# themeshpotato/rust-ray-tracing-in-a-weekend

Hardware: AMD Instinct MI355X
Metric: Msamples/s (pixels x spp) for 1200x800 random-spheres scene (higher is better)
Workload: dtype f64

## Files before the change

__graft_entry__.py:

```python
from __future__ import annotations

import concurrent.futures as cf
import importlib.util
import os
import subprocess
import sys

REPO = os.path.dirname(os.path.abspath(__file__))
PKG = os.path.join(REPO, "rust-ray-tracing-in-a-weekend_amd")
CSRC = os.path.join(PKG, "csrc")
INCLUDE = os.path.join(REPO, "include")
ORACLE = os.path.join(REPO, "oracle")

HIPCC = os.environ.get("HIPCC", "/opt/rocm/bin/hipcc")
ARCH = os.environ.get("RT_OFFLOAD_ARCH", "gfx950")
CXXFLAGS = ["-O3", "-std=c++17", "-fPIC", "-ffp-contract=off", "-fno-fast-math", f"--offload-arch={ARCH}",
            "-I" + INCLUDE, "-Wall", "-Wno-unused-function",
            "-mllvm", "-disable-machine-licm"]
F32_FLAGS = ["-ffp-contract=fast"]
F32_SPHERES_FLAGS = ["-fno-hip-fp32-correctly-rounded-divide-sqrt"]
F32_FINAL_FLAGS = ["-fno-hip-fp32-correctly-rounded-divide-sqrt"]


def tu_flags(src: str, flags=None) -> list:
    flags = list(CXXFLAGS if flags is None else flags)
    name = os.path.basename(src)
    if name.startswith("trace_f32_"):
        flags = [f for f in flags if f != "-ffp-contract=off"] + F32_FLAGS
        if name.startswith("trace_f32_spheres"):
            flags += F32_SPHERES_FLAGS
        if name.startswith("trace_f32_final"):
            flags += F32_FINAL_FLAGS
    return flags


VARIANTS = ["all", "final", "media", "rectinst", "spheres"]
SOURCES = ([f"trace_v_{v}.hip" for v in VARIANTS] + [f"trace_v_{v}_count.hip" for v in VARIANTS] +
           [f"trace_f32_{v}.hip" for v in VARIANTS] + ["trace_f32_final_count.hip", "trace_f32_spheres_count.hip"] +
           [f"features_v_{v}.hip" for v in VARIANTS] +
           ["trace_kernel.hip", "features_kernel.hip", "adaptive_kernel.hip", "adaptive_state_kernel.hip", "denoise_kernel.hip", "atrous_kernel.hip", "cross_kernel.hip", "pyramid_kernel.hip", "scene_model.cpp", "flatten.cpp", "bvh_build.cpp", "scene_lower.cpp",
            "launch_plan.cpp", "deal_cache.cpp", "denoise_host.cpp", "atrous_host.cpp", "cross_host.cpp", "pyramid_host.cpp", "abi.cpp", "abi_scene.cpp",
            "abi_passes.cpp", "abi_adaptive_state.cpp", "adaptive_frame.cpp", "adaptive_schedule.cpp", "abi_filters.cpp", "comm.cpp"])


def _run(cmd):
    r = subprocess.run(cmd, capture_output=True, text=True)
    if r.returncode != 0:
        raise RuntimeError(f"command failed ({r.returncode}): {' '.join(cmd)}\n{r.stdout}\n{r.stderr}")
    return r


def build_library(verbose: bool = False, extra_flags=(), name: str = "librtiow_amd.so", licm: bool = False,
                  csrc: str = CSRC) -> str:
    objdir = os.path.join(PKG, "build" if not (extra_flags or licm or csrc != CSRC) else "build_" + os.path.splitext(name)[0])
    flags = [f for f in CXXFLAGS if not (licm and f in ("-mllvm", "-disable-machine-licm"))]
    libdir = os.path.join(PKG, "lib")
    os.makedirs(objdir, exist_ok=True)
    os.makedirs(libdir, exist_ok=True)

    ident = [f'-DRT_SRC_HASH="{source_hash(extra_flags, licm=licm, csrc=csrc)}"']

    stamp = os.path.join(objdir, "flags.txt")
    flag_line = " ".join(flags + list(extra_flags)) + " | f32: " + " ".join(F32_FLAGS) + " | f32 spheres: " + \
        " ".join(F32_SPHERES_FLAGS) + " | f32 final: " + " ".join(F32_FINAL_FLAGS)
    same_flags = os.path.exists(stamp) and open(stamp).read() == flag_line
    headers = [os.path.join(csrc, f) for f in os.listdir(csrc) if f.endswith(".hpp")] + \
              [os.path.join(INCLUDE, "rt", f) for f in os.listdir(os.path.join(INCLUDE, "rt"))]
    newest_header = max(os.path.getmtime(h) for h in headers)

    def compile_one(src):
        obj = os.path.join(objdir, os.path.splitext(src)[0] + ".o")
        path = os.path.join(csrc, src)
        if (same_flags and src != "abi.cpp" and os.path.exists(obj) and
                os.path.getmtime(obj) > max(os.path.getmtime(path), newest_header)):
            return obj
        lang = [] if src.endswith(".hip") else ["-x", "hip"]
        _run([HIPCC, *lang, *tu_flags(src, flags), *extra_flags, *(ident if src == "abi.cpp" else []), "-c", path,
              "-o", obj])
        return obj

    with cf.ThreadPoolExecutor(max_workers=min(8, os.cpu_count() or 4)) as ex:
        objs = list(ex.map(compile_one, SOURCES))
    open(stamp, "w").write(flag_line)
    out = os.path.join(libdir, name)
    _run([HIPCC, f"--offload-arch={ARCH}", "-shared", "-o", out, *objs, "-ldl"])
    if verbose:
        print("built", out)
    return out


def source_hash(extra_flags=(), licm: bool = False, csrc: str = CSRC) -> str:
    import hashlib
    flags = [f for f in CXXFLAGS if not f.startswith("-I") and not (licm and f in ("-mllvm", "-disable-machine-licm"))]
    h = hashlib.sha256(" ".join(flags + list(extra_flags) + F32_FLAGS + F32_SPHERES_FLAGS + F32_FINAL_FLAGS).encode())
    for d in (csrc, os.path.join(INCLUDE, "rt")):
        for name in sorted(os.listdir(d)):
            if name.endswith((".hip", ".hpp", ".cpp", ".h")):
                h.update(name.encode())
                h.update(open(os.path.join(d, name), "rb").read())
    return h.hexdigest()[:16]


SAN_FLAGS = ["-Xarch_host", "-fsanitize=address", "-Xarch_host", "-fsanitize=undefined",
             "-Xarch_host", "-fno-sanitize-recover=undefined", "-Xarch_host", "-fno-omit-frame-pointer"]
HOST_SOURCES = ["scene_model.cpp", "flatten.cpp", "bvh_build.cpp", "scene_lower.cpp", "launch_plan.cpp", "deal_cache.cpp",
                "denoise_host.cpp", "atrous_host.cpp", "cross_host.cpp", "pyramid_host.cpp", "abi.cpp", "abi_scene.cpp", "abi_passes.cpp",
                "abi_adaptive_state.cpp", "adaptive_frame.cpp", "adaptive_schedule.cpp", "abi_filters.cpp",
                "comm.cpp"]


def build_sanitized() -> tuple:
    objdir = os.path.join(PKG, "build")
    kernel_objs = [os.path.join(objdir, os.path.splitext(s)[0] + ".o") for s in SOURCES if s not in HOST_SOURCES]
    if not all(os.path.exists(o) for o in kernel_objs):
        build_library()
    sandir = os.path.join(PKG, "build_asan")
    os.makedirs(sandir, exist_ok=True)

    ident = [f'-DRT_SRC_HASH="{source_hash()}"']

    def compile_one(src):
        obj = os.path.join(sandir, os.path.splitext(src)[0] + ".o")
        _run([HIPCC, "-x", "hip", *CXXFLAGS, "-O1", "-g", *SAN_FLAGS, *(ident if src == "abi.cpp" else []), "-c",
              os.path.join(CSRC, src), "-o", obj])
        return obj

    with cf.ThreadPoolExecutor(max_workers=3) as ex:
        objs = list(ex.map(compile_one, HOST_SOURCES))
    lib = os.path.join(PKG, "lib", "librtiow_amd_asan.so")
    _run([HIPCC, f"--offload-arch={ARCH}", "-shared", "-o", lib, *objs, *kernel_objs, "-ldl"])
    _run(["make", "-C", ORACLE, "-s", "asan"])
    return lib, os.path.join(ORACLE, "build", "liboracle_asan.so")


def build_oracle() -> str:
    _run(["make", "-C", ORACLE, "-s"])
    return os.path.join(ORACLE, "build", "liboracle.so")


def import_binding():
    if PKG not in sys.path:
        sys.path.insert(0, PKG)
    spec = importlib.util.spec_from_file_location("rtiow_amd", os.path.join(PKG, "rtiow_amd.py"))
    mod = importlib.util.module_from_spec(spec)
    sys.modules["rtiow_amd"] = mod
    spec.loader.exec_module(mod)
    return mod


def build_calib() -> str:
    for name in ("valu_calib", "write_calib"):
        src = os.path.join(REPO, "scripts", "calib", name + ".hip")
        out = os.path.join(REPO, "scripts", "calib", name)
        _run([HIPCC, "-O3", f"--offload-arch={ARCH}", src, "-o", out])
    return os.path.join(REPO, "scripts", "calib", "valu_calib")


def build() -> None:
    build_library()
    build_oracle()
    build_calib()
    rt = import_binding()
    lib = rt.load_library()
    missing = [s for s in rt.EXPORTED if not hasattr(lib, s)]
    if missing:
        raise RuntimeError(f"library is missing exports: {missing}")


def smoke() -> None:
    import numpy as np
    sys.path.insert(0, REPO)
    rt = import_binding()
    from tests import oracle_binding as ob

    W, H, spp = 48, 32, 4
    img, stats = rt.render_scene(0, W, H, spp, max_depth=50, out_format=rt.RT_OUT_F64)
    ref = ob.render(0, W, H, spp, max_depth=50)
    err = float(np.max(np.abs(img - ref)))
    print(f"smoke: random scene {W}x{H}x{spp}: kernel {stats.kernel_ms:.3f} ms, max |gpu - oracle| = {err:.3e}")
    if not err <= 1e-3:
        raise AssertionError(f"GPU render differs from the oracle: L_inf = {err}")


if __name__ == "__main__":
    cmd = sys.argv[1] if len(sys.argv) > 1 else "build"
    {"build": build, "smoke": smoke}[cmd]()
```

include/rt/rt_abi.h:

```cpp
#ifndef RT_ABI_H
#define RT_ABI_H

#include <stddef.h>
#include <stdint.h>

#include "rt_scene.h"

#ifdef __cplusplus
extern "C" {
#endif

#define RT_ABI_VERSION 6

enum {
    RT_OK = 0,
    RT_ERR_INVALID = -1,
    RT_ERR_HIP = -2,
    RT_ERR_UNSUPPORTED = -3,
    RT_ERR_OOM = -4,
    RT_ERR_NO_DEVICE = -5,
    RT_ERR_NO_SCENE = -6,
    RT_ERR_COMM = -7,
    RT_ERR_PEER = -8
};
// ... 53 lines not shown
typedef struct rt_scene_preset {
    double look_from[3], look_at[3], background[3];
    double vfov, aperture, focus_dist, time0, time1;
    int32_t default_width, default_spp;
    double default_aspect;
} rt_scene_preset;
int rt_scene_preset_get(int scene_id, rt_scene_preset* out);
int rt_scene_camera(int scene_id, int width, int height, rt_camera* cam_out, double background_out[3]);

enum {
    RT_BUILD_C_ISECT = 1,
    RT_BUILD_MAX_LEAF = 2,
    RT_BUILD_FORCE_LEAF = 3,
    RT_BUILD_ROOT_LEAF = 4,
    RT_BUILD_SPLIT_BOX_PAIRS = 5,
    RT_BUILD_SPLIT_BLAS_PAIRS = 6,
    RT_BUILD_TIME0 = 7,
    RT_BUILD_TIME1 = 8
};
int rt_world_set_build_option(rt_world* w, int key, double value);
int rt_world_flatten(rt_world* w, int accel, const rt_scene_soa** soa_out);
int rt_scene_validate(const rt_scene_soa* soa, int32_t* tlas_depth, int32_t* blas_depth);
int rt_ctx_upload_soa(rt_ctx* ctx, const rt_scene_soa* soa);
int rt_ctx_upload_world(rt_ctx* ctx, rt_world* w, int accel);

enum { RT_OUT_F32 = 0, RT_OUT_F64 = 1 };

typedef struct rt_render_params {
    int32_t width, height;
    int32_t spp, max_depth;
    int32_t spp_chunk;
    int32_t row_begin, row_stride;
    int32_t out_format;
    int32_t out_on_device;
    int32_t count_work;
    double background[3];
    uint64_t render_seed;
    void* stream;
    int32_t row_block;
    int32_t tile_shard;
} rt_render_params;

int rt_render(rt_ctx* ctx, const rt_camera* cam, const rt_render_params* p, void* out);

int rt_rows_in_shard(int height, int row_begin, int row_stride);
int rt_rows_in_band_shard(int height, int row_begin, int row_stride, int row_block);
int rt_tiles_in_shard(int width, int height, int tile_begin, int tile_stride);

typedef struct rt_stats {
    double kernel_ms;
    double reduce_ms;
    uint64_t samples;
    uint64_t casts;
    uint64_t node_visits;
    uint64_t prim_tests;
    uint64_t n_items;
    int32_t n_chunks, spp_chunk;
    int64_t scene_bytes;
    int32_t node_bytes, prim_bytes, material_bytes;
    int32_t variant_features;
    int32_t slab32;
    int32_t lds_stack;
    int32_t lds_nodes;
    uint64_t cycles_camera;
    uint64_t cycles_trace;
    uint64_t cycles_shade;
    uint64_t wave_steps;
    uint64_t wave_node_steps;
    uint64_t cycles_nodes;
    uint64_t cycles_leaves;
    int32_t schedule;
    int32_t n_batches;
    uint64_t wave_leaf_steps;
    uint64_t camera_lanes;
    uint64_t camera_steps;
    uint64_t shade_lanes;
    uint64_t shade_steps;
    int32_t precision;
    int32_t waves_per_simd;
    int64_t trace_buf_bytes;
    int32_t overlapped;
    int32_t reserved0;
    int64_t ring_bytes;
} rt_stats;
int rt_last_stats(rt_ctx* ctx, rt_stats* out);
int rt_last_counters(rt_ctx* ctx, uint64_t* out, int n);

int rt_last_tile_costs(rt_ctx* ctx, uint64_t* out, int64_t n);
int rt_ctx_set_tile_order(rt_ctx* ctx, const uint32_t* order, int64_t n);
int rt_last_deal_order(rt_ctx* ctx, uint32_t* out, int64_t n);

typedef struct rt_comm rt_comm;
enum { RT_COMM_ID_BYTES = 128 };
int rt_comm_unique_id(uint8_t id[RT_COMM_ID_BYTES]);
int rt_comm_init_rank(rt_ctx* ctx, int rank, int world, const uint8_t id[RT_COMM_ID_BYTES], rt_comm** out);
int rt_comm_init_all(rt_ctx* const* ctxs, int n, rt_comm** comms_out);
void rt_comm_destroy(rt_comm* comm);
int rt_comm_rank(const rt_comm* comm, int* rank, int* world);

int rt_comm_tile_order(rt_comm* comm, const rt_camera* cam, const rt_render_params* p, int cost_spp);
int rt_comm_tile_order_all(rt_comm* const* comms, int n, const rt_camera* cam, const rt_render_params* p,
                           int cost_spp);

int rt_render_gather(rt_comm* comm, const rt_camera* cam, const rt_render_params* p, void* frame);
int rt_render_gather_all(rt_comm* const* comms, int n, const rt_camera* cam, const rt_render_params* p,
                         void* frame);

typedef struct rt_comm_stats {
    double render_ms;
    double gather_ms;
    double assemble_ms;
    double kernel_ms;
    int64_t slab_bytes;
    int32_t tiles;
    int32_t tile_order;
    double cost_pass_ms;
    int32_t peer_failed;
} rt_comm_stats;
int rt_comm_last_stats(rt_comm* comm, rt_comm_stats* out);

int rt_tiles_assemble(rt_ctx* ctx, const void* slabs, int64_t slab_elems, int world, const rt_render_params* p,
                      void* frame);
int rt_tiles_assemble_host(const void* slabs, int64_t slab_elems, int world, int width, int height, int elem_bytes,
                           const uint32_t* order, void* frame);
int rt_cost_tile_order(const uint64_t* costs, int64_t n, uint32_t* order);

typedef struct rt_accum rt_accum;
int rt_accum_create(rt_ctx* ctx, const rt_render_params* p, rt_accum** out);
void rt_accum_destroy(rt_accum* acc);
int rt_accum_add(rt_ctx* ctx, rt_accum* acc, const rt_camera* cam, const rt_render_params* p, int sample_count);
int rt_accum_get(rt_accum* acc, double* sums, int64_t* samples_done);
int rt_accum_set(rt_accum* acc, const double* sums, int64_t samples_done);
int rt_accum_resolve(rt_ctx* ctx, rt_accum* acc, double divisor, int out_format, int out_on_device, void* out);

typedef int (*rt_progress_fn)(void* user, int64_t samples_done, int64_t samples_total);
int rt_render_progressive(rt_ctx* ctx, const rt_camera* cam, const rt_render_params* p, int batch_spp,
                          rt_progress_fn progress, void* user, void* out);

typedef struct rt_adaptive_params {
    int32_t min_spp;
    int32_t step_spp;
    double threshold;
} rt_adaptive_params;

typedef struct rt_adaptive_out {
    void* mean;
    uint32_t* tile_spp;
    double* tile_error;
    double* stderr_map;
} rt_adaptive_out;

int rt_render_adaptive(rt_ctx* ctx, const rt_camera* cam, const rt_render_params* p, const rt_adaptive_params* ap,
                       const rt_adaptive_out* out);

typedef struct rt_adaptive_stats {
    int32_t passes;
    int32_t min_spp, step_spp;
    int32_t spp_chunk;
    int32_t tiles;
    int32_t max_pass_batches;
    uint64_t samples_traced;
    uint64_t samples_uniform;
    double trace_ms;
    double moments_ms;
    double classify_ms;
} rt_adaptive_stats;
int rt_adaptive_last_stats(rt_ctx* ctx, rt_adaptive_stats* out);

// ... 111 lines not shown
    double sigma_albedo, sigma_normal, sigma_depth;
} rt_denoise_guides;
int rt_denoise_guided(rt_ctx* ctx, const rt_denoise_params* p, const void* mean, const double* stderr_map,
                      const rt_denoise_guides* g, void* out);
int rt_denoise_guided_host(const rt_denoise_params* p, const void* mean, const double* stderr_map,
                           const rt_denoise_guides* g, void* out);

typedef struct rt_atrous_params {
    int32_t width, height, format, on_device;
    int32_t levels, demodulate;
    double sigma_l;
    void* stream;
} rt_atrous_params;
int rt_denoise_atrous(rt_ctx* ctx, const rt_atrous_params* p, const void* mean, const double* stderr_map,
                      const rt_denoise_guides* g, void* out, double* stderr_out );
int rt_denoise_atrous_host(const rt_atrous_params* p, const void* mean, const double* stderr_map,
                           const rt_denoise_guides* g, void* out, double* stderr_out );

typedef struct rt_atrous_stats {
    double kernel_ms;
    int32_t levels;
    int64_t scratch_bytes;
} rt_atrous_stats;
int rt_atrous_last_stats(rt_ctx* ctx, rt_atrous_stats* out);

typedef struct rt_cross_params {
    int32_t width, height, format, on_device;
    int32_t radius, patch;
    double k;
    double variance_scale;
    void* stream;
} rt_cross_params;
int rt_denoise_cross(rt_ctx* ctx, const rt_cross_params* p, const void* mean_a, const void* mean_b,
                     const double* stderr_map, const rt_denoise_guides* g , void* out,
                     double* stderr_out );
int rt_denoise_cross_host(const rt_cross_params* p, const void* mean_a, const void* mean_b, const double* stderr_map,
                          const rt_denoise_guides* g , void* out, double* stderr_out );

typedef struct rt_cross_stats {
    double kernel_ms;
    int32_t radius, patch;
    int32_t lds_bytes;
    int32_t reserved0;
    int64_t scratch_bytes;
} rt_cross_stats;
int rt_cross_last_stats(rt_ctx* ctx, rt_cross_stats* out);

typedef struct rt_pyramid_params {
    int32_t width, height, format, on_device;
    int32_t radius, patch;
    double k;
    int32_t levels;
    int32_t reserved0;
    void* stream;
} rt_pyramid_params;
int rt_denoise_pyramid(rt_ctx* ctx, const rt_pyramid_params* p, const void* mean, const double* stderr_map,
                       const rt_denoise_guides* g , void* out);
int rt_denoise_pyramid_host(const rt_pyramid_params* p, const void* mean, const double* stderr_map,
                            const rt_denoise_guides* g , void* out);

typedef struct rt_pyramid_stats {
    double kernel_ms;
    int32_t levels, radius, patch;
    int32_t reserved0;
    int64_t scratch_bytes;
} rt_pyramid_stats;
int rt_pyramid_last_stats(rt_ctx* ctx, rt_pyramid_stats* out);

int rt_write_ppm_f64(const double* rgb, int samples_per_pixel, int width, int height, const char* path);
int rt_write_color(const double* rgb, int samples_per_pixel, int64_t n, int32_t* out);
int rt_write_ppm(const float* mean_rgb, int width, int height, const char* path);

int rt_ctx_set_variant(rt_ctx* ctx, int slab32, int lds_stack, int lds_nodes);

enum {
    RT_OPT_TRACE_BUF_BYTES = 1,
    RT_OPT_BATCH_OVERLAP = 2,
    RT_OPT_BLOCK_SAMPLES = 3,
    RT_OPT_BLOCK_CHUNKS = 4,
    RT_OPT_EXTRA_FEATURES = 5,
    RT_OPT_HOIST = 6,
    RT_OPT_POOL_RING = 9,
    RT_OPT_COMM_DIRECT = 10,
    RT_OPT_AUTO_DEAL_ORDER = 11
};
int rt_ctx_set_option(rt_ctx* ctx, int key, int64_t value);
int rt_ctx_get_option(rt_ctx* ctx, int key, int64_t* value);

enum { RT_SCHED_CHUNKS = 0, RT_SCHED_POOL = 1, RT_SCHED_ITEMS = 2, RT_SCHED_AUTO = 3 };
int rt_ctx_set_schedule(rt_ctx* ctx, int schedule);

enum { RT_PREC_F64 = 0, RT_PREC_F32 = 1 };
int rt_ctx_set_precision(rt_ctx* ctx, int precision);

int rt_device_eval(rt_ctx* ctx, int fn, const double* x, const double* y, const double* z, double* out, int n);

#ifdef __cplusplus
}
#endif
#endif
```

rust-ray-tracing-in-a-weekend_amd/csrc/abi.cpp:

```cpp
#include <hip/hip_runtime.h>

#include <algorithm>
#include <cmath>
#include <cstring>
#include <new>
#include <string>
#include <vector>

#include "rt/rt_abi.h"
#include "rt/rt_numerics.h"
#include "ctx_internal.hpp"
#include "deal_cache.hpp"
#include "launch_plan.hpp"
#include "render_internal.hpp"
#include "scene_lower.hpp"
#include "trace_kernel.hpp"

namespace {

thread_local std::string g_last_error;

}

int rtx::fail(int code, const std::string& msg)
{
    g_last_error = msg;
    return code;
}

int rtx::hip_fail(hipError_t e, const char* what)
{
    return fail(RT_ERR_HIP, std::string(what) + ": " + hipGetErrorString(e));
}

static size_t default_buf_cap()
{
    size_t fr = 0, tot = 0;
    size_t cap = (size_t)64 << 30;
    if (hipMemGetInfo(&fr, &tot) == hipSuccess && fr > 0) cap = std::min(cap, fr / 2);
    return std::max(cap >> 20, (size_t)1) << 20;
}

#ifndef RT_SRC_HASH
#define RT_SRC_HASH "unknown"
#endif

extern "C" {

int rt_abi_version(void) { return RT_ABI_VERSION; }
const char* rt_last_error(void) { return g_last_error.c_str(); }
const char* rt_build_info(void) { return RT_SRC_HASH; }

int rt_device_count(int* count)
{
    if (!count) return fail(RT_ERR_INVALID, "null count");
    int n = 0;
    hipError_t e = hipGetDeviceCount(&n);
    if (e != hipSuccess) {
        *count = 0;
        return hip_fail(e, "hipGetDeviceCount");
    }
    *count = n;
    return RT_OK;
}

int rt_ctx_create(int device, rt_ctx** out)
{
    if (!out) return fail(RT_ERR_INVALID, "null out");
    *out = nullptr;
    int n = 0;
    if (hipGetDeviceCount(&n) != hipSuccess || n <= 0) return fail(RT_ERR_NO_DEVICE, "no HIP device visible");
    if (device < 0 || device >= n) return fail(RT_ERR_INVALID, "device index out of range");
    HIP_TRY(hipSetDevice(device));
    rt_ctx* c = new (std::nothrow) rt_ctx();
    if (!c) return fail(RT_ERR_OOM, "rt_ctx");
    c->device = device;
    c->sample_buf_cap = default_buf_cap();
    {
        int v = 0;
        if (hipDeviceGetAttribute(&v, hipDeviceAttributeMaxSharedMemoryPerMultiprocessor, device) == hipSuccess && v > 0)
            c->dev.lds_per_cu = (size_t)v;
        if (hipDeviceGetAttribute(&v, hipDeviceAttributeMaxSharedMemoryPerBlock, device) == hipSuccess && v > 0)
            c->dev.lds_per_block = (size_t)v;
        if (hipDeviceGetAttribute(&v, hipDeviceAttributeMultiprocessorCount, device) == hipSuccess && v > 0)
            c->dev.n_cus = v;
        c->dev.lds_per_block = std::min(c->dev.lds_per_block, c->dev.lds_per_cu);
    }
    hipError_t e = hipStreamCreateWithFlags(&c->stream, hipStreamNonBlocking);
    for (int i = 0; i < 2 && e == hipSuccess; ++i) e = hipStreamCreateWithFlags(&c->tstream[i], hipStreamNonBlocking);
    if (e == hipSuccess) e = c->ev.create();
    if (e == hipSuccess) e = c->flt_denoise.ev.create();
    if (e == hipSuccess) e = c->ev_ft.create();
    if (e == hipSuccess) e = c->flt_atrous.ev.create();
    if (e == hipSuccess) e = c->flt_cross.ev.create();
    if (e == hipSuccess) e = c->flt_pyramid.ev.create();
    if (e == hipSuccess) e = c->ev_pf.create(hipEventDisableTiming);
    if (e == hipSuccess) e = c->ev_done.create(hipEventDisableTiming);
    if (e == hipSuccess) e = c->ev_in.create(hipEventDisableTiming);
    if (e == hipSuccess) e = c->ev_tr.create(hipEventDisableTiming);
    if (e == hipSuccess) e = c->ev_rd.create(hipEventDisableTiming);
    if (e == hipSuccess) e = c->counters.alloc(kCounters * sizeof(unsigned long long));
    if (e == hipSuccess) e = c->params.alloc(kParamSlots * sizeof(rtk::KParams));
    if (e == hipSuccess) e = c->work.alloc(2 * rtk::kDealTable * sizeof(unsigned));
    if (e != hipSuccess) {
        rt_ctx_destroy(c);
        return hip_fail(e, "rt_ctx_create");
    }
    *out = c;
    return RT_OK;
}

void rt_ctx_destroy(rt_ctx* c)
{
    if (!c) return;
    (void)hipSetDevice(c->device);
    if (c->stream) (void)hipStreamSynchronize(c->stream);
    if (c->ev_done.ev[0] && c->any_enqueued) (void)c->ev_done.wait(0);
    for (hipStream_t s : c->tstream) {
        if (s) (void)hipStreamSynchronize(s);
        if (s) (void)hipStreamDestroy(s);
    }
    if (c->stream) (void)hipStreamDestroy(c->stream);
    delete c;
}

int rt_ctx_upload_soa(rt_ctx* c, const rt_scene_soa* s)
{
    if (!c || !s) return fail(RT_ERR_INVALID, "null argument");
    rtl::Lowered L;
    std::string err;
    const int rc = rtl::lower(*s, c->opt_hoist != 0, L, err);
    if (rc) return fail(rc, err);
    c->upload_gen++;
    c->deal.drop();
    c->last_deal_n = 0;

    struct Table {
        const void* src;
        size_t bytes, off;
    } t[10] = {{L.nodes.data(), L.nodes.size() * sizeof(rt_bvh_node), 0},
               {s->prim_refs, (size_t)s->n_prim_refs * 4, 0},
               {L.prims.data(), L.prims.size() * sizeof(rt_prim), 0},
               {L.instances.data(), L.instances.size() * sizeof(rt_instance), 0},
               {s->materials, (size_t)s->n_materials * sizeof(rt_material), 0},
               {s->textures, (size_t)s->n_textures * sizeof(rt_texture), 0},
               {s->perlin_ranvec, (size_t)s->n_perlin * 768 * 8, 0},
               {s->perlin_perm, (size_t)s->n_perlin * 768 * 4, 0},
               {s->image_data, (size_t)s->image_bytes, 0},
               {L.leaf_prims.data(), L.leaf_prims.size() * sizeof(rt_prim), 0}};
    size_t total = 0;
    for (Table& e : t) {
        e.off = total;
        total = align_up(total + e.bytes, 256);
    }
    total = std::max<size_t>(total, 256);
    HIP_TRY(hipSetDevice(c->device));
    HIP_TRY(hipStreamSynchronize(c->stream));
    if (c->any_enqueued) HIP_TRY(c->ev_done.wait(0));
    const int rc_buf = c->scene_buf.reserve(c->stream, total);
    if (rc_buf) return rc_buf;
    char* base = c->scene_buf.as<char>();
    for (const Table& e : t)
        if (e.bytes) HIP_TRY(hipMemcpy(base + e.off, e.src, e.bytes, hipMemcpyHostToDevice));

    rtk::SceneDev& S = c->S;
    S.nodes = (const rt_bvh_node*)(base + t[0].off);
    S.prim_refs = (const int32_t*)(base + t[1].off);
    S.prims = (const rt_prim*)(base + t[2].off);
    S.instances = (const rt_instance*)(base + t[3].off);
    S.materials = (const rt_material*)(base + t[4].off);
    S.textures = (const rt_texture*)(base + t[5].off);
    S.perlin_ranvec = (const double*)(base + t[6].off);
    S.perlin_perm = (const int32_t*)(base + t[7].off);
    S.image = (const uint8_t*)(base + t[8].off);
    S.leaf_prims = (const rt_prim*)(base + t[9].off);
    S.tlas_root = s->tlas_root;
    S.pre_leaf = L.pre_leaf;
    S.pre_root = L.pre_root;
    std::copy(L.pre_lo, L.pre_lo + 3, S.pre_lo);
    std::copy(L.pre_hi, L.pre_hi + 3, S.pre_hi);
    S.stack16_ok = L.stack16_ok;
    S.blas_base = L.blas_base;
    S.stack_entries = L.stack_entries;
    S.n_tlas_nodes = L.n_tlas_nodes;
    S.n_blas_bfs = L.n_blas_bfs;
    S.n_lds_nodes = S.n_lds_blas = S.seed_stage_bytes = 0;
    S.has_lights = L.has_lights;
    S.has_spheres = L.has_spheres;
    c->scene = rtp::scene_facts(L, *s);
    c->has_scene = true;
    c->stats.scene_bytes = (int64_t)total;
    return RT_OK;
}

int rt_ctx_upload_world(rt_ctx* c, rt_world* w, int accel)
{
    const rt_scene_soa* soa = nullptr;
    int rc = rt_world_flatten(w, accel, &soa);
    if (rc) return rc;
    return rt_ctx_upload_soa(c, soa);
}

int rt_rows_in_shard(int height, int row_begin, int row_stride) { return rtp::rows_in_shard(height, row_begin, row_stride); }
int rt_rows_in_band_shard(int height, int row_begin, int row_stride, int row_block)
{
    return rtp::rows_in_band_shard(height, row_begin, row_stride, row_block);
}
int rt_tiles_in_shard(int width, int height, int tile_begin, int tile_stride)
{
    return rtp::tiles_in_shard(width, height, tile_begin, tile_stride);
}

}

int fill_kparams(rt_ctx* c, const rt_camera* cam, const rt_render_params* p, const Layout& lay, int chunk,
                 const Sink& sink, int64_t img_tiles, rtk::KParams& K)
{
// ... 17 lines not shown
    K.row_block_shift = 0;
    while ((1 << K.row_block_shift) < row_block_of(p)) K.row_block_shift++;
    K.tile_shard = p->tile_shard;
    K.img_tiles_x = (p->width + 7) / 8;
    {
        const uint64_t d = (uint64_t)K.img_tiles_x, m = ((uint64_t)1 << 32) / std::max<uint64_t>(d, 1) + 1;
        const uint64_t e = m * d - ((uint64_t)1 << 32);
        K.tile_div_magic = (d >= 2 && m < ((uint64_t)1 << 32) && (uint64_t)img_tiles * e < ((uint64_t)1 << 32))
                               ? (uint32_t)m : 0u;
    }
    if (sink.moments) {
        K.tile_order = sink.moments->order;
    } else if (p->tile_shard && c->tile_order_n > 0) {
        if (c->tile_order_n != img_tiles)
            return fail(RT_ERR_INVALID, "the tile order has " + std::to_string(c->tile_order_n) + " tiles, the frame " +
                                            std::to_string(img_tiles));
        K.tile_order = c->tile_order.as<uint32_t>();
        K.tile_major = 1;
    }
    K.n_rows = lay.rows;
    K.tiles_x = (lay.w + 7) / 8;
    K.tiles_y = (lay.rows + 7) / 8;
    return RT_OK;
}

static int deal_setup(rt_ctx* c, const rt_camera* cam, const rt_render_params* p, const rtp::Plan& pl, bool adaptive_pass,
                      int64_t img_tiles, hipStream_t stream, rtk::KParams& K)
{
    c->last_deal_n = 0;
    const bool ok = rtk::deal_variant(pl.variant) && rtd::eligible(*p, pl.schedule, adaptive_pass);
    const rtd::Decision d = c->deal.next(c->opt_deal, ok, rtd::key_of(c->upload_gen, *cam, *p), img_tiles);
    const size_t n = (size_t)img_tiles;
    if (d.measure) {
        if (img_tiles > c->deal_cap) {
            HIP_TRY(hipStreamSynchronize(stream));
            const size_t stride = rtk::kDealTable + 2 * n;
            DevBuf w;
            const hipError_t e = w.alloc(2 * stride * sizeof(unsigned));
            if (e != hipSuccess) {
                c->deal.drop();
                return hip_fail(e, "deal order table");
            }
            c->work = std::move(w);
            c->work_stride = stride;
            c->deal_cap = img_tiles;
        }
        std::vector<uint32_t> raster(n);
        for (size_t i = 0; i < n; ++i) raster[i] = (uint32_t)i;
        for (int h = 0; h < 2; ++h) {
            unsigned* t = c->work.as<unsigned>() + h * c->work_stride + rtk::kDealTable;
            HIP_TRY(hipMemcpyAsync(t, raster.data(), n * sizeof(uint32_t), hipMemcpyHostToDevice, stream));
            HIP_TRY(hipMemsetAsync(t + n, 0, n * sizeof(unsigned), stream));
        }
        HIP_TRY(hipStreamSynchronize(stream));
        K.tile_major = rtk::kDealMeasure;
    }
    if (d.build) {
        std::vector<uint32_t> part(2 * n);
        hipError_t e = hipSuccess;
        for (int h = 0; h < 2 && e == hipSuccess; ++h)
            e = hipMemcpyAsync(part.data() + h * n, c->work.as<unsigned>() + h * c->work_stride + rtk::kDealTable + n, n * sizeof(uint32_t),
                               hipMemcpyDeviceToHost, stream);
        if (e == hipSuccess) e = hipStreamSynchronize(stream);
        if (e != hipSuccess) {
            c->deal.fail_build();
            return hip_fail(e, "deal order: tile costs");
        }
        std::vector<uint64_t> costs(n);
        for (size_t i = 0; i < n; ++i) costs[i] = (uint64_t)part[i] + part[n + i];
        const std::vector<uint32_t>& order = c->deal.finish_build(costs.data());
        for (int h = 0; h < 2 && e == hipSuccess; ++h)
            e = hipMemcpyAsync(c->work.as<unsigned>() + h * c->work_stride + rtk::kDealTable, order.data(), n * sizeof(uint32_t),
                               hipMemcpyHostToDevice, stream);
        if (e == hipSuccess) e = hipStreamSynchronize(stream);
        if (e != hipSuccess) {
            c->deal.fail_build();
            return hip_fail(e, "deal order: upload");
        }
    }
    if (d.ordered) {
        K.tile_major = rtk::kDealOrdered;
        c->last_deal_n = img_tiles;
    }
    return RT_OK;
}

static void write_stats(rt_ctx* c, const rtp::Plan& pl, int chunk, int waves_per_simd, bool count)
{
    rt_stats& st = c->stats;
    st.lds_nodes = pl.n_lds_nodes;
    st.variant_features = (int32_t)pl.variant;
    st.slab32 = pl.slab32;
    st.lds_stack = pl.lds_stack;
    st.schedule = pl.schedule;
    st.precision = pl.f32 ? RT_PREC_F32 : RT_PREC_F64;
    st.waves_per_simd = waves_per_simd;
    st.n_batches = pl.n_batches;
    st.ring_bytes = (int64_t)pl.ring_bytes;
    st.trace_buf_bytes = (int64_t)pl.trace_buf_bytes;
    st.overlapped = pl.overlap ? 1 : 0;
    st.n_chunks = pl.n_chunks;
    st.samples = (uint64_t)pl.px * (uint64_t)pl.total;
    st.n_items = (uint64_t)pl.px * (uint64_t)pl.n_chunks;
    st.spp_chunk = chunk;
    st.node_bytes = (int32_t)sizeof(rt_bvh_node);
    st.prim_bytes = (int32_t)sizeof(rt_prim);
    st.material_bytes = (int32_t)sizeof(rt_material);
    c->ev.arm();
    c->pending_counts = count;
    if (!st.samples) st.casts = st.node_visits = st.prim_tests = 0;
}

int run_range(rt_ctx* c, const rt_camera* cam, const rt_render_params* p, int s_begin, int s_end, int chunk,
              hipStream_t stream, const Sink& sink)
{
    const Layout lay = layout_of(p);
    const long long n_px = (long long)lay.rows * lay.w;
    if (n_px == 0 || s_end <= s_begin) {
        for (int i = 0; i < 3; ++i) HIP_TRY(c->ev.record(i, stream));
        write_stats(c, rtp::Plan{}, chunk, 0, false);
        c->last_deal_n = 0;
        return RT_OK;
    }

    const int64_t img_tiles = (int64_t)((p->width + 7) / 8) * ((p->height + 7) / 8);
    rtk::KParams K;
    int rc = fill_kparams(c, cam, p, lay, chunk, sink, img_tiles, K);
    if (rc) return rc;

    rtp::Request rq;
    rq.lay = lay;
    rq.s_begin = s_begin;
    rq.s_end = s_end;
    rq.chunk = chunk;
    rq.count_work = p->count_work != 0;
    rq.acc_sink = sink.acc != nullptr;
    rq.moments = sink.moments != nullptr;
    rq.cam_mag = rtp::camera_magnitude(*cam);
    rq.cam_time0 = cam->time0;
    rq.cam_time1 = cam->time1;
    rtp::Retry retry{c->sample_buf_cap, true};
    rtp::Plan pl;
    for (;;) {
        pl = rtp::plan(c->scene, c->dev, c->opt, rq, retry);
        if (pl.err) return fail(pl.err, pl.err_msg);
        rc = c->acc_tmp.reserve(stream, pl.acc_bytes);
        if (rc) return rc;
        bool oom = false;
        rc = c->partial.reserve(stream, pl.partial_bytes, &oom);
        if (rc == RT_OK && pl.ring) {
            rc = c->ring.reserve(stream, pl.ring_bytes, &oom);
            if (rc != RT_OK && oom) {
                retry.ring_allowed = false;
                continue;
            }
        }
        if (rc == RT_OK) break;
        if (!oom) return rc;
        if (!rtp::shrink(pl, retry)) return hip_fail(hipErrorOutOfMemory, "trace output buffer (smallest batch)");
    }
    double* const acc_tmp = c->acc_tmp.as<double>();
    double* const open = pl.open_chunk ? acc_tmp : nullptr;
    double* const acc = !pl.own_total ? sink.acc : pl.open_chunk ? acc_tmp + pl.px * 3 : acc_tmp;
    PlannedLaunch launch = planned_launch(c->S, pl);
    const rtk::SceneDev& S = launch.S;
    K.block_chunks = pl.block_chunks;
    K.block_samples = pl.block_samples;
    K.ring_waves = pl.ring_waves;
    int waves_per_simd = 0;
    rtk::LaunchOpts& o = launch.o;
    o.count = rq.count_work;
    o.waves_per_simd = &waves_per_simd;
    const rtk::SampleTiles tiles{lay.w, lay.rows, (lay.w + 7) / 8, pl.f32};
    rc = deal_setup(c, cam, p, pl, sink.moments != nullptr, img_tiles, stream, K);
    if (rc) return rc;

    if (pl.own_total) HIP_TRY(hipMemsetAsync(acc, 0, pl.px_bytes, stream));
    if (rq.count_work) {
        HIP_TRY(hipMemsetAsync(c->counters.p, 0, kCounters * sizeof(unsigned long long), stream));
        rc = c->tile_cost.reserve(stream, (size_t)img_tiles * sizeof(unsigned long long));
        if (rc) return rc;
        HIP_TRY(hipMemsetAsync(c->tile_cost.p, 0, (size_t)img_tiles * sizeof(unsigned long long), stream));
        K.tile_cost = c->tile_cost.as<unsigned long long>();
        c->tile_cost_n = pl.schedule == RT_SCHED_POOL || pl.schedule == RT_SCHED_ITEMS ? img_tiles : 0;
    }
    HIP_TRY(c->ev.record(0, stream));
    if (pl.overlap) {
        HIP_TRY(c->ev_in.record(0, stream));
        for (int i = 0; i < 2; ++i) HIP_TRY(hipStreamWaitEvent(c->tstream[i], c->ev_in.ev[0], 0));
    }
    for (int bi = 0; bi < pl.n_batches; ++bi) {
        const int b0 = s_begin + (int)(bi * pl.batch);
        const int b1 = (int)std::min<long long>(s_end, b0 + pl.batch);
        K.sample_begin = b0;
        K.spp = b1;
        K.n_chunks = (b1 - b0 + chunk - 1) / chunk;
        {
            const bool items = pl.schedule == RT_SCHED_ITEMS;
            const unsigned g = items ? (unsigned)K.block_chunks : (unsigned)K.block_samples;
            const unsigned n = items ? (unsigned)K.n_chunks : (unsigned)(K.spp - K.sample_begin);
            const unsigned n_groups = (n + g - 1) / std::max(g, 1u);
            K.n_work_blocks = (unsigned)K.tiles_x * (unsigned)K.tiles_y * n_groups;
            K.deal_div = K.tile_major ? n_groups : (unsigned)K.tiles_x * (unsigned)K.tiles_y;
        }
        const int h = pl.overlap ? (bi & 1) : 0;
        double* buf = c->partial.as<double>() + (size_t)h * (pl.half_bytes / sizeof(double));
        hipStream_t ts = pl.overlap ? c->tstream[h] : stream;
        K.ring = pl.ring ? c->ring.as<double>() + (size_t)h * (pl.ring_one_bytes / sizeof(double)) : nullptr;
        if (pl.overlap && bi >= 2) HIP_TRY(hipStreamWaitEvent(ts, c->ev_rd.ev[h], 0));
        rtk::KParams* dK = c->params.as<rtk::KParams>() + c->param_slot;
        c->param_slot = (c->param_slot + 1) % kParamSlots;
        HIP_TRY(hipMemcpyAsync(dK, &K, sizeof K, hipMemcpyHostToDevice, ts));
        HIP_TRY(rtk::launch_trace(S, K, dK, buf, c->counters.as<unsigned long long>(),
                                  c->work.as<unsigned>() + h * c->work_stride, o, ts));
        if (bi == pl.n_batches - 1) HIP_TRY(c->ev.record(1, ts));
        if (pl.overlap) {
            HIP_TRY(c->ev_tr.record(h, ts));
            HIP_TRY(hipStreamWaitEvent(stream, c->ev_tr.ev[h], 0));
        }
        if (sink.moments) {
            HIP_TRY(rtk::launch_adaptive_moments(buf, *sink.moments, K.tiles_x, b1 - b0, chunk,
                                                 (int)(((long long)b0 - s_begin) % chunk), bi == pl.n_batches - 1,
                                                 sink.n_done, stream, sink.halves, b0));
        } else if (!pl.per_sample) {
            if (acc) HIP_TRY(rtk::launch_accumulate(buf, acc, n_px, K.n_chunks, stream));
            else HIP_TRY(rtk::launch_reduce(buf, sink.out, sink.f64, n_px, K.n_chunks, sink.scale, stream));
        } else if (!open) {
            HIP_TRY(rtk::launch_reduce_samples(buf, sink.out, sink.f64, tiles, b1 - b0, chunk, sink.scale, stream));
        } else {
            HIP_TRY(rtk::launch_reduce_samples_carry(buf, acc, open, tiles, b1 - b0, chunk,
                                                     (int)(((long long)b0 - s_begin) % chunk), bi == pl.n_batches - 1,
                                                     stream));
        }
        if (pl.overlap) HIP_TRY(c->ev_rd.record(h, stream));
    }
    if (pl.own_total)
        HIP_TRY(rtk::launch_reduce(acc, sink.out, sink.f64, n_px, 1, sink.scale, stream));
    HIP_TRY(c->ev.record(2, stream));
    write_stats(c, pl, chunk, waves_per_simd, rq.count_work);
    return RT_OK;
}

extern "C" {

int rt_render(rt_ctx* c, const rt_camera* cam, const rt_render_params* p, void* out)
{
    if (!c || !cam || !p || !out) return fail(RT_ERR_INVALID, "null argument");
    if (!c->has_scene) return fail(RT_ERR_NO_SCENE, "no scene uploaded");
    if (bad_geometry(p) || p->spp < 1 || p->max_depth < 0 || (p->out_format != RT_OUT_F32 && p->out_format != RT_OUT_F64))
        return fail(RT_ERR_INVALID, "bad render params");
    const Layout lay = layout_of(p);
    const int chunk = p->spp_chunk > 0 ? std::min(p->spp_chunk, p->spp) : auto_chunk(p->spp);
    const long long n_px = (long long)lay.rows * lay.w;

    HIP_TRY(hipSetDevice(c->device));
    hipStream_t stream = p->stream ? (hipStream_t)p->stream : c->stream;
    StreamScope scope(c, stream);
// ... 230 lines not shown
    for (int64_t i = 0; i < n; ++i) {
        if ((int64_t)order[i] >= n || seen[order[i]]) return fail(RT_ERR_INVALID, "the tile order is not a permutation of 0..n-1");
        seen[order[i]] = 1;
    }
    HIP_TRY(hipSetDevice(c->device));
    HIP_TRY(hipDeviceSynchronize());
    c->tile_order.release();
    c->tile_order_n = 0;
    if (n == 0) return RT_OK;
    HIP_TRY(c->tile_order.alloc((size_t)n * sizeof(uint32_t)));
    HIP_TRY(hipMemcpy(c->tile_order.p, order, (size_t)n * sizeof(uint32_t), hipMemcpyHostToDevice));
    c->tile_order_n = n;
    return RT_OK;
}

int rt_last_deal_order(rt_ctx* c, uint32_t* out, int64_t n)
{
    if (!c || (!out && n > 0) || n < 0) return fail(RT_ERR_INVALID, "bad argument");
    if (c->last_deal_n == 0) return 0;
    const std::vector<uint32_t>& order = c->deal.order();
    const int64_t m = std::min<int64_t>(n, (int64_t)order.size());
    if (m > 0) std::memcpy(out, order.data(), (size_t)m * sizeof(uint32_t));
    return (int)c->last_deal_n;
}

int rt_last_counters(rt_ctx* c, uint64_t* out, int n)
{
    if (!c || !out || n < 0) return fail(RT_ERR_INVALID, "null argument");
    rt_stats st;
    const int rc = rt_last_stats(c, &st);
    if (rc) return rc;
    for (int i = 0; i < n; ++i) out[i] = i < kCounters ? (uint64_t)c->raw_counters[i] : 0;
    return std::min(n, kCounters);
}

int rt_ctx_set_variant(rt_ctx* c, int slab32, int lds_stack, int lds_nodes)
{
    if (!c || slab32 < 0 || slab32 > 1 || lds_stack < 0 || lds_stack > 1 || lds_nodes < 0 || lds_nodes > 1)
        return fail(RT_ERR_INVALID, "bad variant");
    c->opt.slab32 = slab32;
    c->opt.lds_stack = lds_stack;
    c->opt.lds_nodes = lds_nodes;
    return RT_OK;
}

int rt_ctx_set_precision(rt_ctx* c, int precision)
{
    if (!c || (precision != RT_PREC_F64 && precision != RT_PREC_F32)) return fail(RT_ERR_INVALID, "bad precision");
    c->opt.precision = precision;
    return RT_OK;
}

int rt_ctx_set_option(rt_ctx* c, int key, int64_t v)
{
    if (!c) return fail(RT_ERR_INVALID, "null context");
    switch (key) {
    case RT_OPT_TRACE_BUF_BYTES:
        if (v < 0) return fail(RT_ERR_INVALID, "negative buffer bound");
        c->sample_buf_cap = v == 0 ? default_buf_cap() : std::max<size_t>((size_t)v, (size_t)1 << 20);
        return RT_OK;
    case RT_OPT_BATCH_OVERLAP: c->opt.overlap = v != 0; return RT_OK;
    case RT_OPT_BLOCK_SAMPLES:
        if (v < 0 || v > 1024) return fail(RT_ERR_INVALID, "block samples out of range (0..1024)");
        c->opt.block_samples = (int)v;
        return RT_OK;
    case RT_OPT_BLOCK_CHUNKS:
        if (v < 0 || v > 64) return fail(RT_ERR_INVALID, "block chunks out of range (0..64)");
        c->opt.block_chunks = (int)v;
        return RT_OK;
    case RT_OPT_EXTRA_FEATURES:
        if (v < 0 || (v & ~(int64_t)rtk::FEAT_ALL)) return fail(RT_ERR_INVALID, "unknown feature bits");
        c->opt.extra_features = (uint32_t)v;
        return RT_OK;
    case RT_OPT_HOIST: c->opt_hoist = v != 0; return RT_OK;
    case RT_OPT_POOL_RING:
        if (v < 0 || v > 2) return fail(RT_ERR_INVALID, "pool ring mode out of range (0 never, 1 when needed, 2 always)");
        c->opt.ring = (int)v;
        return RT_OK;
    case RT_OPT_COMM_DIRECT: c->opt_comm_direct = v != 0; return RT_OK;
    case RT_OPT_AUTO_DEAL_ORDER:
        if (v < 0 || v > 2) return fail(RT_ERR_INVALID, "deal order mode out of range (0 off, 1 auto, 2 measure only)");
        c->opt_deal = (int)v;
        return RT_OK;
    default: return fail(RT_ERR_INVALID, "unknown option");
    }
}

int rt_ctx_get_option(rt_ctx* c, int key, int64_t* v)
{
    if (!c || !v) return fail(RT_ERR_INVALID, "null argument");
    switch (key) {
    case RT_OPT_TRACE_BUF_BYTES: *v = (int64_t)c->sample_buf_cap; return RT_OK;
    case RT_OPT_BATCH_OVERLAP: *v = c->opt.overlap; return RT_OK;
    case RT_OPT_BLOCK_SAMPLES: *v = c->opt.block_samples; return RT_OK;
    case RT_OPT_BLOCK_CHUNKS: *v = c->opt.block_chunks; return RT_OK;
    case RT_OPT_EXTRA_FEATURES: *v = c->opt.extra_features; return RT_OK;
    case RT_OPT_HOIST: *v = c->opt_hoist; return RT_OK;
    case RT_OPT_POOL_RING: *v = c->opt.ring; return RT_OK;
    case RT_OPT_COMM_DIRECT: *v = c->opt_comm_direct; return RT_OK;
    case RT_OPT_AUTO_DEAL_ORDER: *v = c->opt_deal; return RT_OK;
    default: return fail(RT_ERR_INVALID, "unknown option");
    }
}

int rt_ctx_set_schedule(rt_ctx* c, int schedule)
{
    if (c && schedule == 4)
        return fail(RT_ERR_UNSUPPORTED, "schedule 4 (wavefront) was removed: 2.3x slower than the pool on C4 (DESIGN.md 5.7)");
    if (!c || schedule < RT_SCHED_CHUNKS || schedule > RT_SCHED_AUTO) return fail(RT_ERR_INVALID, "bad schedule");
    c->opt.schedule = schedule;
    return RT_OK;
}

int rt_device_eval(rt_ctx* c, int fn, const double* x, const double* y, const double* z, double* out, int n)
{
    if (!c || !x || !out || n < 0 || fn < 0 || fn > 13) return fail(RT_ERR_INVALID, "bad argument");
    if (n == 0) return RT_OK;
    HIP_TRY(hipSetDevice(c->device));
    DevBuf blk;
    const size_t b = (size_t)n * sizeof(double);
    HIP_TRY(blk.alloc(4 * b));
    double* const d = blk.as<double>();
    hipError_t e = hipMemcpy(d, x, b, hipMemcpyHostToDevice);
    if (e == hipSuccess) e = hipMemcpy(d + n, y ? y : x, b, hipMemcpyHostToDevice);
    if (e == hipSuccess) e = hipMemcpy(d + 2 * n, z ? z : x, b, hipMemcpyHostToDevice);
    if (e == hipSuccess) e = rtk::launch_eval(fn, d, d + n, d + 2 * n, d + 3 * n, n, c->stream);
    if (e == hipSuccess) e = hipStreamSynchronize(c->stream);
    if (e == hipSuccess) e = hipMemcpy(out, d + 3 * n, b, hipMemcpyDeviceToHost);
    if (e != hipSuccess) return hip_fail(e, "rt_device_eval");
    return RT_OK;
}

}
```

rust-ray-tracing-in-a-weekend_amd/csrc/abi_scene.cpp:

```cpp
#include <algorithm>
#include <cmath>
#include <cstdio>
#include <new>
#include <string>
#include <vector>

#include "rt/rt_abi.h"
#include "rt/rt_numerics.h"
#include "ctx_internal.hpp"
#include "scene_lower.hpp"
#include "scene_model.hpp"

struct rt_world {
    explicit rt_world(uint64_t seed) : w(seed) {}
    rtw::World w;
};

extern "C" {

int rt_world_create(uint64_t scene_seed, rt_world** out)
{
    if (!out) return fail(RT_ERR_INVALID, "null out");
    *out = new (std::nothrow) rt_world(scene_seed);
    return *out ? RT_OK : fail(RT_ERR_OOM, "rt_world");
}
void rt_world_destroy(rt_world* w) { delete w; }

#define CHECK_WORLD(w, o)                                              \
    do {                                                               \
        if (!(w) || !(o)) return fail(RT_ERR_INVALID, "null argument"); \
    } while (0)

static rtw::V3 vec(const double* a) { return rtw::v3(a[0], a[1], a[2]); }

int rt_world_texture_solid(rt_world* w, double r, double g, double b, int* o)
{
    CHECK_WORLD(w, o);
    *o = w->w.texture_solid(rtw::v3(r, g, b));
    return RT_OK;
}
int rt_world_texture_checker(rt_world* w, const double even[3], const double odd[3], int* o)
{
    CHECK_WORLD(w, o);
    if (!even || !odd) return fail(RT_ERR_INVALID, "null color");
    *o = w->w.texture_checker(vec(even), vec(odd));
    return RT_OK;
}
int rt_world_texture_noise(rt_world* w, double scale, int* o)
{
    CHECK_WORLD(w, o);
    *o = w->w.texture_noise(scale);
    return RT_OK;
}
int rt_world_texture_image(rt_world* w, const uint8_t* rgb, int width, int height, int* o)
{
    CHECK_WORLD(w, o);
    if (width < 0 || height < 0 || (!rgb && width * height > 0)) return fail(RT_ERR_INVALID, "bad image");
    *o = w->w.texture_image(rgb, width, height);
    return RT_OK;
}

int rt_world_material_lambertian(rt_world* w, int tex, int* o)
{
    CHECK_WORLD(w, o);
    if (!w->w.valid_texture(tex)) return fail(RT_ERR_INVALID, "bad texture id");
    *o = w->w.lambertian(tex);
    return RT_OK;
}
int rt_world_material_metal(rt_world* w, const double albedo[3], double fuzz, int* o)
{
    CHECK_WORLD(w, o);
    if (!albedo) return fail(RT_ERR_INVALID, "null albedo");
    *o = w->w.metal(vec(albedo), fuzz);
    return RT_OK;
}
int rt_world_material_dielectric(rt_world* w, double ir, int* o)
{
    CHECK_WORLD(w, o);
    *o = w->w.dielectric(ir);
    return RT_OK;
}
int rt_world_material_diffuse_light(rt_world* w, int tex, int* o)
{
    CHECK_WORLD(w, o);
    if (!w->w.valid_texture(tex)) return fail(RT_ERR_INVALID, "bad texture id");
    *o = w->w.diffuse_light(tex);
    return RT_OK;
}
int rt_world_material_isotropic(rt_world* w, int tex, int* o)
{
    CHECK_WORLD(w, o);
    if (!w->w.valid_texture(tex)) return fail(RT_ERR_INVALID, "bad texture id");
// ... 128 lines not shown
                  double aspect, double aperture, double focus_dist, double t0, double t1, rt_camera* out)
{
    if (!look_from || !look_at || !vup || !out) return fail(RT_ERR_INVALID, "null argument");
    *out = rtw::camera_new(vec(look_from), vec(look_at), vec(vup), vfov, aspect, aperture, focus_dist, t0, t1);
    return RT_OK;
}

int rt_scene_preset_get(int scene_id, rt_scene_preset* out)
{
    if (!out) return fail(RT_ERR_INVALID, "null out");
    rtw::Preset p;
    if (!rtw::scene_preset(scene_id, p)) return fail(RT_ERR_INVALID, "unknown scene id");
    auto put = [](double* d, rtw::V3 a) { d[0] = a.x; d[1] = a.y; d[2] = a.z; };
    put(out->look_from, p.look_from);
    put(out->look_at, p.look_at);
    put(out->background, p.background);
    out->vfov = p.vfov;
    out->aperture = 0.1;
    out->focus_dist = 10.0;
    out->time0 = 0.0;
    out->time1 = 1.0;
    out->default_width = p.width;
    out->default_spp = p.spp;
    out->default_aspect = p.aspect;
    return RT_OK;
}

int rt_scene_camera(int scene_id, int width, int height, rt_camera* cam, double bg[3])
{
    if (!cam || width < 1 || height < 1) return fail(RT_ERR_INVALID, "bad argument");
    rtw::Preset p;
    if (!rtw::scene_preset(scene_id, p)) return fail(RT_ERR_INVALID, "unknown scene id");
    *cam = rtw::camera_new(p.look_from, p.look_at, rtw::v3(0.0, 1.0, 0.0), p.vfov, (double)width / (double)height,
                           0.1, 10.0, 0.0, 1.0);
    if (bg) {
        bg[0] = p.background.x;
        bg[1] = p.background.y;
        bg[2] = p.background.z;
    }
    return RT_OK;
}

int rt_world_set_build_option(rt_world* w, int key, double v)
{
    if (!w) return fail(RT_ERR_INVALID, "null world");
    if (!std::isfinite(v)) return fail(RT_ERR_INVALID, "build option value not finite");
    rtw::BuildOptions& b = w->w.build;
    const int iv = v < 0 ? -1 : (int)std::min(v, 1e6);
    switch (key) {
    case RT_BUILD_C_ISECT: b.c_isect = v > 0 ? v : 0.0; return RT_OK;
    case RT_BUILD_MAX_LEAF: b.max_leaf = std::max(iv, 0); return RT_OK;
    case RT_BUILD_FORCE_LEAF: b.force_leaf = std::max(iv, 0); return RT_OK;
    case RT_BUILD_ROOT_LEAF: b.root_leaf = iv; return RT_OK;
    case RT_BUILD_SPLIT_BOX_PAIRS: b.split_box_pairs = iv; return RT_OK;
    case RT_BUILD_SPLIT_BLAS_PAIRS: b.split_blas_pairs = iv; return RT_OK;
    case RT_BUILD_TIME0: b.time0 = v; return RT_OK;
    case RT_BUILD_TIME1: b.time1 = v; return RT_OK;
    default: return fail(RT_ERR_INVALID, "unknown build option");
    }
}

int rt_world_flatten(rt_world* w, int accel, const rt_scene_soa** soa_out)
{
    if (!w || !soa_out) return fail(RT_ERR_INVALID, "null argument");
    std::string err;
    int rc = rtw::flatten(w->w, accel, err);
    if (rc) return fail(rc, err);
    *soa_out = &w->w.flat.soa;
    return RT_OK;
}

int rt_scene_validate(const rt_scene_soa* s, int32_t* tlas_depth, int32_t* blas_depth)
{
    if (!s) return fail(RT_ERR_INVALID, "null argument");
    int t = 0, b = 0, n = 0;
    std::string err;
    const int rc = rtl::validate(*s, t, b, n, err);
    if (rc) return fail(rc, err);
    if (tlas_depth) *tlas_depth = t;
    if (blas_depth) *blas_depth = b;
    return RT_OK;
}

static inline int write_color_f64(double x, double scale)
{
    const double r = std::sqrt(x * scale);
    const double c = r < 0.0 ? 0.0 : r > 0.999 ? 0.999 : r;
    return (int)rt_sat_i32(256.0 * c);
}

int rt_write_color(const double* rgb, int samples_per_pixel, int64_t n, int32_t* out)
{
    if (!rgb || !out || n < 0 || samples_per_pixel < 1) return fail(RT_ERR_INVALID, "bad argument");
    const double scale = 1.0 / (double)samples_per_pixel;
    for (int64_t i = 0; i < 3 * n; ++i) out[i] = write_color_f64(rgb[i], scale);
    return RT_OK;
}

int rt_write_ppm_f64(const double* rgb, int samples_per_pixel, int width, int height, const char* path)
{
    if (!rgb || !path || width < 1 || height < 1 || samples_per_pixel < 1) return fail(RT_ERR_INVALID, "bad argument");
    FILE* f = std::fopen(path, "wb");
    if (!f) return fail(RT_ERR_INVALID, std::string("cannot open ") + path);
    const double scale = 1.0 / (double)samples_per_pixel;
    std::fprintf(f, "P3\n%d %d\n255\n\n", width, height);
    for (int j = height - 1; j >= 0; --j)
        for (int i = 0; i < width; ++i) {
            const double* px = rgb + ((size_t)j * width + i) * 3;
            std::fprintf(f, "%d %d %d\n", write_color_f64(px[0], scale), write_color_f64(px[1], scale),
                         write_color_f64(px[2], scale));
        }
    if (std::fclose(f) != 0) return fail(RT_ERR_INVALID, std::string("cannot write ") + path);
    return RT_OK;
}

int rt_write_ppm(const float* mean, int width, int height, const char* path)
{
    if (!mean || !path || width < 1 || height < 1) return fail(RT_ERR_INVALID, "bad argument");
    FILE* f = std::fopen(path, "wb");
    if (!f) return fail(RT_ERR_INVALID, std::string("cannot open ") + path);
    std::fprintf(f, "P3\n%d %d\n255\n\n", width, height);
    auto to_byte = [](double x) {
        double r = std::sqrt(x);
        double c = r < 0.0 ? 0.0 : r > 0.999 ? 0.999 : r;
        return (int)rt_sat_i32(256.0 * c);
    };
    for (int j = height - 1; j >= 0; --j)
        for (int i = 0; i < width; ++i) {
            const float* px = mean + ((size_t)j * width + i) * 3;
            std::fprintf(f, "%d %d %d\n", to_byte(px[0]), to_byte(px[1]), to_byte(px[2]));
        }
    std::fclose(f);
    return RT_OK;
}

}
```

rust-ray-tracing-in-a-weekend_amd/csrc/ctx_internal.hpp:

```cpp
#pragma once

#include <hip/hip_runtime.h>

#include <cstddef>
#include <cstdint>
#include <string>

#include "rt/rt_abi.h"
#include "deal_cache.hpp"
#include "launch_plan.hpp"
#include "trace_kernel.hpp"

namespace rtx {

int fail(int code, const std::string& msg);
int hip_fail(hipError_t e, const char* what);

}

using rtx::fail;
using rtx::hip_fail;

#define HIP_TRY(expr)                                   \
    do {                                                \
// ... 66 lines not shown
    {
        for (hipEvent_t e : ev)
            if (e) (void)hipEventDestroy(e);
    }

    hipError_t create(unsigned flags = hipEventDefault)
    {
        hipError_t e = hipSuccess;
        for (int i = 0; i < N && e == hipSuccess; ++i) e = hipEventCreateWithFlags(&ev[i], flags);
        return e;
    }
    hipError_t record(int i, hipStream_t stream) { return hipEventRecord(ev[i], stream); }
    hipError_t wait(int i) { return hipEventSynchronize(ev[i]); }
    hipError_t elapsed(int i, float* ms) { return hipEventElapsedTime(ms, ev[i], ev[i + 1]); }
    void arm() { pending = true; }
    void disarm() { pending = false; }
    int resolve(float ms[N - 1])
    {
        if (!pending) return RT_OK;
        HIP_TRY(wait(N - 1));
        for (int i = 0; i + 1 < N; ++i) HIP_TRY(elapsed(i, &ms[i]));
        pending = false;
        return RT_OK;
    }
};

template <typename Stats>
struct FilterSlot {
    Stats stats{};
    EventSpan<2> ev;
    DevBuf scratch;
};

using rtk::kCounters;

struct rt_ctx {
    int device = 0;
    hipStream_t stream = nullptr;
    DevBuf scene_buf;
    rtk::SceneDev S{};
    bool has_scene = false;
    DevBuf partial;
    DevBuf out_buf;
    DevBuf counters;
    DevBuf params;
    int param_slot = 0;
    EventSpan<3> ev;
    EventSpan<1> ev_done;
    hipStream_t last_stream = nullptr;
    bool any_enqueued = false;
    bool pending_counts = false;
    rt_stats stats{};
    rt_adaptive_stats astats{};
    FilterSlot<rt_denoise_stats> flt_denoise;
    rt_features_stats fstats{};
    EventSpan<3> ev_ft;
    FilterSlot<rt_atrous_stats> flt_atrous;
    FilterSlot<rt_cross_stats> flt_cross;
    FilterSlot<rt_pyramid_stats> flt_pyramid;
    EventSpan<2> ev_pf;
    rtp::SceneFacts scene;
    rtp::DeviceFacts dev;
    rtp::Options opt;
    int opt_comm_direct = 1;
    DevBuf ring;
    unsigned long long raw_counters[kCounters] = {};
    DevBuf tile_order;
    int64_t tile_order_n = 0;
    DevBuf tile_cost;
    int64_t tile_cost_n = 0;
    int opt_hoist = 1;
    size_t sample_buf_cap = (size_t)32 << 30;
    DevBuf work;
    size_t work_stride = rtk::kDealTable;
    hipStream_t tstream[2] = {nullptr, nullptr};
    EventSpan<1> ev_in;
    EventSpan<2> ev_tr, ev_rd;
    DevBuf acc_tmp;
    int opt_deal = rtd::kAuto;
    uint64_t upload_gen = 0;
    rtd::DealCache deal;
    int64_t deal_cap = 0;
    int64_t last_deal_n = 0;
};

struct StreamScope {
    rt_ctx* c;
    hipStream_t stream;
    bool open = false;
    StreamScope(rt_ctx* c_, hipStream_t s_) : c(c_), stream(s_) {}
    int begin()
    {
        if (c->any_enqueued && stream != c->last_stream) HIP_TRY(hipStreamWaitEvent(stream, c->ev_done.ev[0], 0));
        open = true;
        return RT_OK;
    }
    int end()
    {
        open = false;
        HIP_TRY(c->ev_done.record(0, stream));
        c->last_stream = stream;
        c->any_enqueued = true;
        return RT_OK;
    }
    ~StreamScope()
    {
        if (open) (void)end();
    }
};

#pragma GCC visibility pop
```

rust-ray-tracing-in-a-weekend_amd/csrc/trace_kernel.hip:

```cpp
#include "trace_launch.hpp"

namespace rtk {

__device__ __forceinline__ bool tile_slot(SampleTiles g, int n_samples, long long i, long long& px, size_t& rec)
{
    const long long tile = i >> 6;
    const int lp = (int)(i & 63);
    const int x = (int)(tile % g.tiles_x) * 8 + (lp & 7);
    const int k = (int)(tile / g.tiles_x) * 8 + (lp >> 3);
    if (x >= g.width || k >= g.n_rows) return false;
    px = (long long)k * g.width + x;
    rec = tiled_record(g.tiles_x, n_samples, x, k, 0);
    return true;
}

constexpr int kReduceWaves = 8;
template <typename T, typename Rec = double>
__global__ void __launch_bounds__(64 * kReduceWaves) reduce_samples_tiled(const Rec* __restrict__ samples,
                                                                          T* __restrict__ out, SampleTiles g,
                                                                          int n_samples, int chunk, double scale)
{
    __shared__ double part[kReduceWaves][3][64];
    const unsigned tile = blockIdx.x;
    const int lane = (int)(threadIdx.x & 63u), w = (int)(threadIdx.x >> 6);
// ... 147 lines not shown
    const int n_r = (int)((n_tiles - r + world - 1) / world);
    const int k = (int)(j / (8LL * n_max));
    const int col = (int)(j - (long long)k * 8 * n_max);
    const int m = col >> 3;
    if (m >= n_r) return;
    const long long pos = r + (long long)m * world;
    const long long t = order ? (long long)order[pos] : pos;
    const int x = (int)(t % tiles_x) * 8 + (col & 7);
    const int y = (int)(t / tiles_x) * 8 + k;
    if (x >= width || y >= height) return;
    const T* src = gathered + (long long)r * slab_elems + ((long long)k * 8 * n_r + col) * 3;
    T* dst = frame + ((long long)y * width + x) * 3;
    dst[0] = src[0];
    dst[1] = src[1];
    dst[2] = src[2];
}

struct StoredUV {
    static constexpr uint32_t F = FEAT_ALL;
};

__global__ void eval_numerics(int fn, const double* x, const double* y, const double* z, double* out, int n)
{
    const int i = blockIdx.x * blockDim.x + threadIdx.x;
    if (i >= n) return;
    double r = 0.0;
    switch (fn) {
    case 0: r = rt_sin(x[i]); break;
    case 1: r = rt_cos(x[i]); break;
    case 2: r = rt_log(x[i]); break;
    case 3: r = rt_atan2(x[i], y[i]); break;
    case 4: r = rt_acos(x[i]); break;
    case 5: case 6: {
        HitT<double> h;
        h.uvkind = 1;
        h.uv0 = x[i]; h.uv1 = y[i]; h.uv2 = z[i];
        double u, v;
        hit_uv<StoredUV>(h, u, v);
        r = fn == 5 ? u : v;
        break;
    }
    case 7: r = rt_pow5(x[i]); break;
    case 8: r = __builtin_sqrt(x[i]); break;
    case 9: r = x[i] / y[i]; break;
    case 10: r = rt_unit53(rt_f64_bits(x[i])); break;
    case 11: r = rt_uniform_sample(rt_f64_bits(x[i]), -1.0, rt_uniform_incl_scale(-1.0, 1.0)); break;
    case 12: r = (double)rt_sin_sign(x[i]); break;
    case 13: r = div_rcp(x[i], y[i], rcp_for_div(y[i])); break;
    default: break;
    }
    out[i] = r;
}

template <bool COUNT, bool F32>
static hipError_t launch_kind(uint32_t f, const Launch& L, const LaunchOpts& o, hipStream_t stream)
{
    switch (f) {
    case FEAT_SET_SPHERES: return launch_variant<FEAT_SET_SPHERES, COUNT, F32>(L, o, stream);
    case FEAT_SET_FINAL: return launch_variant<FEAT_SET_FINAL, COUNT, F32>(L, o, stream);
    }
    if constexpr (COUNT && F32) {
        return hipErrorNotSupported;
    } else {
        switch (f) {
        case FEAT_SET_RECTINST: return launch_variant<FEAT_SET_RECTINST, COUNT, F32>(L, o, stream);
        case FEAT_SET_MEDIA: return launch_variant<FEAT_SET_MEDIA, COUNT, F32>(L, o, stream);
        default: return launch_variant<FEAT_ALL, COUNT, F32>(L, o, stream);
        }
    }
}

hipError_t launch_trace(const SceneDev& S, const KParams& Ph, const KParams* P, double* out,
                        unsigned long long* counters, unsigned* work, const LaunchOpts& o, hipStream_t stream)
{
    Launch L;
    L.S = &S;
    L.P = P;
    L.out = out;
    L.counters = counters;
    L.work = work;
    L.pool = o.pool;
    L.waves_per_simd = o.waves_per_simd;
    L.max_waves = o.pool == 1 && Ph.ring ? (unsigned)Ph.ring_waves : 0u;
    const long long groups = o.pool == 2   ? (Ph.n_chunks + std::max(1, Ph.block_chunks) - 1) / std::max(1, Ph.block_chunks)
                             : o.pool == 1 ? ((long long)Ph.spp - Ph.sample_begin + std::max(1, Ph.block_samples) - 1) /
                                                 std::max(1, Ph.block_samples)
                                           : Ph.n_chunks;
    L.n_blocks = (unsigned long long)Ph.tiles_x * Ph.tiles_y * groups;
    if (L.n_blocks == 0) return hipSuccess;
    if (L.n_blocks > 0xfffffff0ULL) return hipErrorInvalidValue;
    if (o.pool) {
        const hipError_t e = hipMemsetAsync(work, 0, sizeof(unsigned), stream);
        if (e != hipSuccess) return e;
    }
    const uint32_t f = variant_features(o.features);
    if (o.f32) return o.count ? launch_kind<true, true>(f, L, o, stream) : launch_kind<false, true>(f, L, o, stream);
    return o.count ? launch_kind<true, false>(f, L, o, stream) : launch_kind<false, false>(f, L, o, stream);
}

hipError_t launch_reduce_samples(const double* samples, void* out, bool f64, SampleTiles g, int n_samples,
                                 int chunk, double scale, hipStream_t stream)
{
    const long long tiles = (long long)tiled_pixels(g.width, g.n_rows) / 64;
    const float* rec32 = reinterpret_cast<const float*>(samples);
    if (tiles <= 0 || chunk < 1) return tiles <= 0 ? hipSuccess : hipErrorInvalidValue;
    const dim3 grid((unsigned)tiles), block(64 * kReduceWaves);
    if (g.f32_records && f64)
        hipLaunchKernelGGL((reduce_samples_tiled<double, float>), grid, block, 0, stream, rec32, (double*)out, g,
                           n_samples, chunk, scale);
    else if (g.f32_records)
        hipLaunchKernelGGL((reduce_samples_tiled<float, float>), grid, block, 0, stream, rec32, (float*)out, g,
                           n_samples, chunk, scale);
    else if (f64)
        hipLaunchKernelGGL(reduce_samples_tiled<double>, grid, block, 0, stream, samples, (double*)out, g, n_samples,
                           chunk, scale);
    else
        hipLaunchKernelGGL(reduce_samples_tiled<float>, grid, block, 0, stream, samples, (float*)out, g, n_samples,
                           chunk, scale);
    return hipGetLastError();
}

hipError_t launch_reduce_samples_carry(const double* samples, double* acc, double* open, SampleTiles g,
                                       int n_samples, int chunk, int pos, bool close, hipStream_t stream)
{
    const long long n_slots = (long long)tiled_pixels(g.width, g.n_rows);
    const long long blocks = (n_slots + 255) / 256;
    if (blocks <= 0) return hipSuccess;
    if (g.f32_records)
        hipLaunchKernelGGL(reduce_samples_carry<float>, dim3((unsigned)blocks), dim3(256), 0, stream,
                           reinterpret_cast<const float*>(samples), acc, open, g, n_slots, n_samples, chunk, pos,
                           (int)close);
    else
        hipLaunchKernelGGL(reduce_samples_carry<double>, dim3((unsigned)blocks), dim3(256), 0, stream, samples, acc,
                           open, g, n_slots, n_samples, chunk, pos, (int)close);
    return hipGetLastError();
}

hipError_t launch_reduce(const double* partial, void* out, bool f64, long long n_px, int n_chunks, double scale,
                         hipStream_t stream)
{
    const long long blocks = (n_px + 255) / 256;
    if (blocks <= 0) return hipSuccess;
    if (f64)
        hipLaunchKernelGGL(reduce_chunks<double>, dim3((unsigned)blocks), dim3(256), 0, stream, partial, (double*)out,
                           n_px, n_chunks, scale);
    else
        hipLaunchKernelGGL(reduce_chunks<float>, dim3((unsigned)blocks), dim3(256), 0, stream, partial, (float*)out,
                           n_px, n_chunks, scale);
    return hipGetLastError();
}

hipError_t launch_accumulate(const double* partial, double* acc, long long n_px, int n_chunks, hipStream_t stream)
{
    const long long blocks = (n_px + 255) / 256;
    if (blocks <= 0) return hipSuccess;
    hipLaunchKernelGGL(accumulate_chunks, dim3((unsigned)blocks), dim3(256), 0, stream, partial, acc, n_px, n_chunks);
    return hipGetLastError();
}

hipError_t launch_assemble_tiles(const void* gathered, void* frame, bool f64, int world, long long slab_elems,
                                 int width, int height, const uint32_t* order, hipStream_t stream)
{
    const int tiles_x = (width + 7) / 8;
    const long long n_tiles = (long long)tiles_x * ((height + 7) / 8);
    const int n_max = (int)((n_tiles + world - 1) / world);
    const long long n = 64LL * n_max * world;
// ... 22 lines not shown
```

rust-ray-tracing-in-a-weekend_amd/csrc/trace_kernel.hpp:

```cpp
#pragma once

#include <hip/hip_runtime.h>

#include "rt/rt_scene.h"
#include "scene_features.hpp"
#include "launch_shapes.hpp"

namespace rtk {

struct SceneDev {
    const rt_prim* prims;
    const int32_t* prim_refs;
    const rt_prim* leaf_prims;
    const rt_bvh_node* nodes;
    const rt_instance* instances;
    const rt_material* materials;
    const rt_texture* textures;
    const double* perlin_ranvec;
    const int32_t* perlin_perm;
    const uint8_t* image;
    int32_t tlas_root;
    int32_t blas_base;
    int32_t stack_entries;
    int32_t n_lds_nodes;
    int32_t n_tlas_nodes;
    int32_t has_spheres;
    int32_t has_lights;
    int32_t n_lds_materials;
    int32_t n_lds_textures;
    int32_t pre_leaf, pre_root;
    float pre_lo[3], pre_hi[3];
    int32_t stack16_ok;
    int32_t n_blas_bfs, n_lds_blas;
    int32_t seed_stage_bytes;
};

struct KParams {
    rt_camera cam;
    double bg[3];
    double scale_m11;
    double scale_time;
    double wm1, hm1;
    double inv_wm1, inv_hm1;
    uint64_t seed;
    int32_t width, height, spp, max_depth;
    int32_t spp_chunk, n_chunks;
    int32_t row_begin, row_stride, n_rows;
    int32_t row_block_shift;
    int32_t tiles_x, tiles_y;
    int32_t sample_begin;
    int32_t block_chunks;
    int32_t block_samples;
    uint32_t n_work_blocks;
    int32_t img_width;
    int32_t tile_shard;
    int32_t img_tiles_x;
    uint32_t tile_div_magic;
    int32_t ring_waves;
    double* ring;
    const uint32_t* tile_order;
    int32_t tile_major;
    uint32_t deal_div;
    unsigned long long* tile_cost;
};

constexpr int32_t kDealOrdered = 2, kDealMeasure = 3;
constexpr unsigned kDealTable = 16;
constexpr bool deal_variant(uint32_t variant) { return variant == FEAT_SET_SPHERES; }

struct LaunchOpts {
    uint32_t features;
    int slab32;
    int lds_stack;
    int count;
    int pool;
    int f32;
    int* waves_per_simd = nullptr;
};

enum CounterSlot : int {
    kCtrCasts = 0,
    kCtrNodeVisits = 1,
    kCtrPrimTests = 2,
    kCtrCyclesCamera = 3,
    kCtrCyclesTrace = 4,
    kCtrCyclesShade = 5,
    kCtrWaveSteps = 6,
    kCtrWaveNodeSteps = 7,
    kCtrCyclesNodes = 8,
    kCtrCyclesLeaves = 9,
    kCtrWaveLeafSteps = 10,
    kCtrCameraLanes = 11,
    kCtrCameraSteps = 12,
    kCtrShadeLanes = 13,
    kCtrShadeSteps = 14,
    kCtrCyclesSetup = 15,
    kCtrCyclesPre = 16,
    kCtrCyclesRecord = 17,
    kCtrCyclesMedia = 18,
    kCtrCyclesInstances = 19,
    kCtrCyclesRefill = 20,
    kCtrCyclesKernel = 21,
    kCtrCyclesDeferred = 22,
    kCtrCyclesSeed = 23,
    kCtrCyclesTries = 24,
    kCtrLongestWave = 25,
    kCtrWaves = 26,
    kCtrIdleTail = 27,
    kCtrIdleRing = 28,
    kCtrNoScatter = 29,
    kCtrDepthCap = 30,
    kCtrTryWait = 31,
};
constexpr int kCounters = kCtrTryWait + 1;
static_assert(kCounters == 32, "rt_last_counters documents 32 slots");

struct SampleTiles {
    int32_t width, n_rows, tiles_x;
    int32_t f32_records;
};
__host__ __device__ inline size_t tiled_record(int tiles_x, int n_samples, int x, int k, int s)
{
    const size_t tile = (size_t)(k >> 3) * (size_t)tiles_x + (size_t)(x >> 3);
    return (tile * (size_t)n_samples + (size_t)s) * 64 + (size_t)(((k & 7) << 3) | (x & 7));
}

hipError_t launch_trace(const SceneDev& S, const KParams& Ph, const KParams* P, double* out,
                        unsigned long long* counters, unsigned* work, const LaunchOpts& o, hipStream_t stream);
hipError_t launch_reduce_samples(const double* samples, void* out, bool f64, SampleTiles g, int n_samples,
                                 int chunk, double scale, hipStream_t stream);
hipError_t launch_reduce_samples_carry(const double* samples, double* acc, double* open, SampleTiles g,
                                       int n_samples, int chunk, int pos, bool close, hipStream_t stream);
hipError_t launch_reduce(const double* partial, void* out, bool f64, long long n_px, int n_chunks, double scale,
                         hipStream_t stream);
hipError_t launch_accumulate(const double* partial, double* acc, long long n_px, int n_chunks, hipStream_t stream);
hipError_t launch_assemble_tiles(const void* gathered, void* frame, bool f64, int world, long long slab_elems,
                                 int width, int height, const uint32_t* order, hipStream_t stream);
hipError_t launch_eval(int fn, const double* x, const double* y, const double* z, double* out, int n,
                       hipStream_t stream);

struct AdaptiveFrame {
    double* sum;
    double* sum_open;
    double* q;
    double* q_open;
    double* tile_error;
    uint32_t* tile_spp;
    const uint32_t* order;
    int32_t width, height, tiles_x, pos_begin;
};
struct AdaptiveHalves {
    double* sum_a;
    double* sum_a_open;
    double* sum_b;
    double* sum_b_open;
};
hipError_t launch_adaptive_moments(const double* samples, const AdaptiveFrame& F, int n_tiles, int n_samples,
                                   int chunk, int pos, bool close, int n_done, hipStream_t stream,
                                   const AdaptiveHalves* halves = nullptr, int first = 0);
hipError_t launch_adaptive_resolve(const double* sum, const double* q, const uint32_t* tile_spp, void* mean, bool f64,
                                   double* se_map, int width, int height, hipStream_t stream);
hipError_t launch_adaptive_resolve_halves(const double* sum_a, const double* sum_b, const uint32_t* tile_spp,
                                          void* mean_a, void* mean_b, bool f64, int width, int height,
                                          hipStream_t stream);

}
```

rust-ray-tracing-in-a-weekend_amd/csrc/trace_launch.hpp:

```cpp
#pragma once
#include "trace_device.hpp"
#include "trace_launch_common.hpp"

namespace rtk {

template <uint32_t F, bool COUNT, bool F32 = false>
hipError_t launch_variant(const Launch& L, const LaunchOpts& o, hipStream_t stream)
{
    const SceneDev& S = *L.S;
    KernelShape k = launch_shape(F, F32, S, o);
    if constexpr (!F32) {
        if (k.s16) {
            using C = Cfg<F, true, true, true, COUNT, false>;
            static const bool static_lds =
                any_static_lds({(const void*)trace_pool<C, false>, (const void*)trace_pool<C, true>,
                                (const void*)trace_pool<C, false, true>, (const void*)trace_chunks<C>}) ||
                [] {
                    if constexpr (RT_STAGE_SEEDS != 0 && C::SHAPE.s16)
                        return any_static_lds({(const void*)trace_pool<CfgStage<C>, false>, (const void*)trace_pool<CfgStage<C>, false, true>});
                    else return false;
                }();
            if (static_lds) k = without_stack16(k);
        }
    }
    const int bt = k.block_threads, wpb = bt / 64;
    const int seed_bytes = RT_STAGE_SEEDS && k.s16 && !F32 && L.pool == 1 && S.seed_stage_bytes == (int)seed_stage_bytes_of(bt)
                               ? S.seed_stage_bytes : 0;
    const size_t lds = launch_lds_bytes(k, S, seed_bytes);
    with_cfg<F, COUNT, F32>(k, [&](auto whole, auto part) {
        using C1 = decltype(whole);
        using C0 = decltype(part);
        if (L.pool) {
            auto go = [&](auto kernel) {
                unsigned nb = std::min<unsigned long long>(resident_blocks(L, kernel, lds, bt), (L.n_blocks + wpb - 1) / wpb);
                if (L.max_waves) nb = std::max(1u, std::min(nb, L.max_waves / (unsigned)wpb));
                hipLaunchKernelGGL(kernel, dim3(nb), dim3(bt), lds, stream, S, L.P, L.out, L.counters, L.work);
            };
            if constexpr (RT_STAGE_SEEDS != 0 && C1::SHAPE.s16 && !F32) {
                if (seed_bytes) return go(L.max_waves ? trace_pool<CfgStage<C1>, false, true> : trace_pool<CfgStage<C1>, false>);
            }
            if (L.pool == 2) go(k.nall ? trace_pool<C1, true> : trace_pool<C0, true>);
            else if (L.max_waves)
                go(k.nall ? trace_pool<C1, false, true> : trace_pool<C0, false, true>);
            else go(k.nall ? trace_pool<C1, false> : trace_pool<C0, false>);
            return;
        }
        const auto kernel = k.nall ? trace_chunks<C1> : trace_chunks<C0>;
        if (L.waves_per_simd) (void)blocks_per_cu(L, kernel, lds, bt);
        hipLaunchKernelGGL(kernel, dim3((unsigned)((L.n_blocks + wpb - 1) / wpb)), dim3(bt), lds, stream, S, L.P, L.out, L.counters);
    });
    return hipGetLastError();
}

#define RT_VARIANT_DECL(F, COUNT, F32) \
    extern template hipError_t launch_variant<F, COUNT, F32>(const Launch&, const LaunchOpts&, hipStream_t);
RT_VARIANT_DECL(FEAT_SET_SPHERES, false, false)
RT_VARIANT_DECL(FEAT_SET_SPHERES, true, false)
RT_VARIANT_DECL(FEAT_SET_RECTINST, false, false)
RT_VARIANT_DECL(FEAT_SET_RECTINST, true, false)
RT_VARIANT_DECL(FEAT_SET_MEDIA, false, false)
RT_VARIANT_DECL(FEAT_SET_MEDIA, true, false)
RT_VARIANT_DECL(FEAT_SET_FINAL, false, false)
RT_VARIANT_DECL(FEAT_SET_FINAL, true, false)
RT_VARIANT_DECL(FEAT_ALL, false, false)
RT_VARIANT_DECL(FEAT_ALL, true, false)
RT_VARIANT_DECL(FEAT_SET_SPHERES, false, true)
RT_VARIANT_DECL(FEAT_SET_RECTINST, false, true)
RT_VARIANT_DECL(FEAT_SET_MEDIA, false, true)
RT_VARIANT_DECL(FEAT_SET_FINAL, false, true)
RT_VARIANT_DECL(FEAT_ALL, false, true)
RT_VARIANT_DECL(FEAT_SET_SPHERES, true, true)
RT_VARIANT_DECL(FEAT_SET_FINAL, true, true)
#undef RT_VARIANT_DECL

}
```

rust-ray-tracing-in-a-weekend_amd/csrc/trace_launch_common.hpp:

```cpp
#pragma once
#include "trace_types.hpp"

namespace rtk {

struct Launch {
    const SceneDev* S;
    const KParams* P;
    double* out;
    unsigned long long* counters;
    unsigned* work;
    int pool;
    unsigned long long n_blocks;
    int* waves_per_simd;
    unsigned max_waves = 0;
};

template <class K>
static int blocks_per_cu(const Launch& L, K kernel, size_t lds, int bt)
{
    int per_cu = 0;
    if (hipOccupancyMaxActiveBlocksPerMultiprocessor(&per_cu, kernel, bt, lds) != hipSuccess || per_cu <= 0) per_cu = 1;
    if (L.waves_per_simd) *L.waves_per_simd = per_cu * (bt / 256);
    return per_cu;
}

template <class K>
static unsigned resident_blocks(const Launch& L, K kernel, size_t lds, int bt)
{
    static int cus = 0;
    if (!cus) {
        int dev = 0;
        (void)hipGetDevice(&dev);
        if (hipDeviceGetAttribute(&cus, hipDeviceAttributeMultiprocessorCount, dev) != hipSuccess || cus <= 0) cus = 256;
    }
    return (unsigned)(cus * blocks_per_cu(L, kernel, lds, bt));
}

inline KernelShape launch_shape(uint32_t F, bool f32, const SceneDev& S, const LaunchOpts& o)
{
    return launch_shape(F, f32 || o.slab32 != 0, o.lds_stack != 0, f32, S.n_lds_nodes, S.n_tlas_nodes, S.stack16_ok != 0);
}

inline size_t launch_lds_bytes(const KernelShape& k, const SceneDev& S, int seed_bytes = 0)
{
    const size_t rest = lds_layout(k, S.n_lds_nodes, S.n_lds_blas, S.stack_entries, S.n_lds_materials, S.n_lds_textures).total;
    return seed_bytes ? lds_seeds_offset(rest) + (size_t)seed_bytes : rest;
}

inline bool any_static_lds(std::initializer_list<const void*> kernels)
{
    hipFuncAttributes a;
    for (const void* k : kernels)
        if (hipFuncGetAttributes(&a, k) != hipSuccess || a.sharedSizeBytes != 0) return true;
    return false;
}
inline KernelShape without_stack16(const KernelShape& k) { return kernel_shape(k.features, k.s32, k.lds, false, k.f32); }

template <uint32_t F, bool COUNT, bool F32, class Fn>
static void with_cfg(const KernelShape& k, Fn fn)
{
    if (k.s32) {
        if (k.lds) fn(Cfg<F, true, true, true, COUNT, F32>{}, Cfg<F, true, true, false, COUNT, F32>{});
        else fn(Cfg<F, true, false, true, COUNT, F32>{}, Cfg<F, true, false, false, COUNT, F32>{});
    } else if constexpr (!F32) {
        if (k.lds) fn(Cfg<F, false, true, true, COUNT, F32>{}, Cfg<F, false, true, false, COUNT, F32>{});
        else fn(Cfg<F, false, false, true, COUNT, F32>{}, Cfg<F, false, false, false, COUNT, F32>{});
    }
}

}
```

rust-ray-tracing-in-a-weekend_amd/csrc/trace_pool.hpp:

```cpp
#pragma once
#include "trace_shade.hpp"
#include "trace_grid.hpp"

namespace rtk {

template <class R>
__device__ __forceinline__ void forget(HitT<R>& h)
{
    h.t = __builtin_nondeterministic_value(h.t);
    h.px = __builtin_nondeterministic_value(h.px);
    h.py = __builtin_nondeterministic_value(h.py);
    h.pz = __builtin_nondeterministic_value(h.pz);
    h.nx = __builtin_nondeterministic_value(h.nx);
    h.ny = __builtin_nondeterministic_value(h.ny);
    h.nz = __builtin_nondeterministic_value(h.nz);
    h.uv0 = __builtin_nondeterministic_value(h.uv0);
    h.uv1 = __builtin_nondeterministic_value(h.uv1);
    h.uv2 = __builtin_nondeterministic_value(h.uv2);
    h.uv3 = __builtin_nondeterministic_value(h.uv3);
    h.front = __builtin_nondeterministic_value(h.front);
    h.mat = __builtin_nondeterministic_value(h.mat);
    h.uvkind = __builtin_nondeterministic_value(h.uvkind);
}

__device__ __forceinline__ unsigned lanes_below(uint64_t mask)
{
    return __builtin_amdgcn_mbcnt_hi((uint32_t)(mask >> 32), __builtin_amdgcn_mbcnt_lo((uint32_t)mask, 0u));
}

#ifndef RING_LOADS
#define RING_LOADS 4
#endif
__device__ __forceinline__ int ring_set(int val, int q, int v) { return (int)__lane_id() == q ? val : v; }

template <class C>
__device__ __forceinline__ double* ring_of_wave(const KParams& P)
{
    const unsigned wave = __builtin_amdgcn_readfirstlane(blockIdx.x * (unsigned)(BlockThreads<C>() / 64) + threadIdx.x / 64u);
    return P.ring + (size_t)wave * kRingWaveDoubles;
}
__device__ __forceinline__ unsigned* ring_block_id(double* ring_wave)
{
    return reinterpret_cast<unsigned*>(ring_wave + (size_t)kPoolRing * kRingSlot * 3);
}
template <class C>
constexpr bool RingSgpr() { return C::F == FEAT_SET_SPHERES; }
template <class C>
constexpr bool DealCfg() { return deal_variant(C::F) && !C::COUNT; }

struct alignas(32) SeedSlot {
    rt_pstream st;
    double u, v;
};
static_assert(sizeof(SeedSlot) == kSeedSlotBytes, "a staged sample start is one slot");
template <class C, bool ITEMS>
constexpr bool StagedPool()
{
    static_assert(!C::STAGE || (Stack16Cfg<C>() && RingSgpr<C>() && !C::F32), "staged sample starts: the f64 spheres variant's 16-bit-stack kernels");
    return C::STAGE && !ITEMS;
}
template <class C>
__device__ __forceinline__ SeedSlot* seed_slots(const SceneDev& S)
{
    return reinterpret_cast<SeedSlot*>(reinterpret_cast<char*>(rt_lds) + lds_seeds_offset(lds_layout_of<C>(S).total));
}

__device__ __forceinline__ void ring_reduce(const KParams& P, const double* __restrict__ rec,
                                            double* __restrict__ partial, unsigned blk, unsigned n_tiles, unsigned group,
                                            size_t n_px, int lane)
{
    const unsigned outer = blk / P.deal_div, inner = blk - outer * P.deal_div;
    const unsigned grp = P.tile_major ? inner : outer, tile = P.tile_major ? outer : inner;
    const int s0 = P.sample_begin + (int)(grp * group);
    const int x = (int)(tile % (unsigned)P.tiles_x) * 8 + (lane & 7);
    const int k = (int)(tile / (unsigned)P.tiles_x) * 8 + (lane >> 3);
    const int ns = min(P.spp, s0 + (int)group) - s0;
    __builtin_amdgcn_fence(__ATOMIC_RELEASE, "workgroup");
    __builtin_amdgcn_fence(__ATOMIC_ACQUIRE, "workgroup");
    constexpr int NB = RING_LOADS;
    const bool own = x < P.width && k < P.n_rows;
    double* o = partial + ((size_t)grp * n_px + (size_t)k * P.width + x) * 3;
#pragma unroll 1
    for (int c = 0; c < 3; ++c) {
        const double* p = rec + (size_t)lane * 3 + c;
        double a = 0.0;
#pragma unroll 1
        for (int j0 = 0; j0 < ns; j0 += NB) {
            double v[NB];
#pragma unroll
            for (int j = 0; j < NB; ++j) v[j] = j0 + j < ns ? p[(size_t)j * 64 * 3] : 0.0;
#pragma unroll
            for (int j = 0; j < NB; ++j)
                if (j0 + j < ns) a = a + v[j];
            p += (size_t)NB * 64 * 3;
        }
        if (own) o[c] = a;
    }
}

template <class C, bool ITEMS, bool RING = false>
__global__ void __launch_bounds__(BlockThreads<C>(), min_waves<C>()) trace_pool(SceneDev S, const KParams* __restrict__ Pp,
                                                                  double* __restrict__ samples,
                                                                  unsigned long long* __restrict__ counters,
                                                                  unsigned* __restrict__ work)
{
    const KParams& P = *Pp;
    stage_lds<C>(S);
    StackT<C> stack;
    if constexpr (Stack16Cfg<C>()) stack.base = reinterpret_cast<short*>(rt_lds + lds_stack_offset<C>(S)) + threadIdx.x;
    else if constexpr (C::LDS) stack.init((int)lds_stack_offset<C>(S));
    Count cnt{};
    uint64_t t_cam = 0, t_trace = 0, t_shade = 0, t_prev = 0, t_start = 0, t_sample = 0;
    if (C::COUNT) t_prev = t_start = __builtin_amdgcn_s_memtime();
    (void)t_trace;
    (void)t_start;
    (void)t_sample;
    const int lane = threadIdx.x & 63;
    const unsigned n_tiles = (unsigned)P.tiles_x * (unsigned)P.tiles_y;
    const unsigned group = ITEMS ? (unsigned)P.block_chunks : (unsigned)P.block_samples;
    const unsigned n_blocks = P.n_work_blocks;
    const size_t n_px = (size_t)P.n_rows * (size_t)P.width;
    unsigned blk_units = 0, blk_next = 0, nvalid = 1;
    int tx0 = 0, tk0 = 0, vw = 1, s0 = 0;
    bool exhausted = false;
    bool active = false, new_sample = false;
    int x = 0, k = 0, s = 0, depth = 0;
    int left = 0;
    bool own = false;
    using R = typename C::Real;
    double cr = 0, cg = 0, cb = 0;
    R Tr = 1, Tg = 1, Tb = 1;
    Keyed key{P.seed, 0, 0, 0};
    rt_pstream st;
    RayT<R> r;
    HitT<R> h;
    bool pending = false;
    bool cam_wait = false;
    (void)cam_wait;
    constexpr bool ring = RING && !ITEMS;
    int ringv = 0;
    unsigned occ = 0, cur_slot = 0;
    for (;;) {
        if constexpr (ring && !RingSgpr<C>()) {
            unsigned occv = (unsigned)__builtin_amdgcn_readlane(ringv, kRingOcc);
            if (occv != 0) {
                const unsigned open = blk_next < blk_units ? (unsigned)__builtin_amdgcn_readlane(ringv, kRingCur) : 99u;
#pragma unroll
                for (int q = 0; q < kPoolRing; ++q) {
                    if ((occv >> q & 1u) && (unsigned)q != open &&
                        __ballot(active && ((unsigned)s >> kRingSampleBits) / kRingSlot == (unsigned)q) == 0) {
                        ring_reduce(P, ring_of_wave<C>(P) + (size_t)q * kRingSlot * 3, samples,
                                    (unsigned)__builtin_amdgcn_readlane(ringv, q), n_tiles, group, n_px, lane);
                        occv &= ~(1u << q);
                        ringv = ring_set((int)occv, kRingOcc, ringv);
                    }
                }
            }
        }
        if (ring && RingSgpr<C>()) {
            if (occ != 0) {
                const unsigned open = blk_next < blk_units ? cur_slot : 99u;
#pragma unroll
                for (int q = 0; q < kPoolRing; ++q) {
                    if ((occ >> q & 1u) && (unsigned)q != open &&
                        __ballot(active && ((unsigned)s >> kRingSampleBits) / kRingSlot == (unsigned)q) == 0) {
                        double* rw = ring_of_wave<C>(P);
                        ring_reduce(P, rw + (size_t)q * kRingSlot * 3, samples,
                                    (unsigned)__builtin_amdgcn_readfirstlane(ring_block_id(rw)[q]), n_tiles, group, n_px, lane);
                        occ &= ~(1u << q);
                    }
                }
            }
        }
        if (ITEMS && own) {
            own = false;
            active = true;
            new_sample = true;
            s += 1;
            left -= 1;
// ... 109 lines not shown
                }
                const unsigned take = min(min((unsigned)__popcll(need), nvalid - col), blk_units - blk_next);
                if (!active && rank < take) {
                    const unsigned p = col + rank;
                    if (nvalid == 64u) {
                        x = tx0 + (int)(p & 7u);
                        k = tk0 + (int)(p >> 3);
                    } else {
                        x = tx0 + (int)(p % (unsigned)vw);
                        k = tk0 + (int)(p / (unsigned)vw);
                    }
                    s = s0 + (int)row;
                    if (ring) s |= (int)((cur_slot * kRingSlot + row * 64u + (unsigned)((k & 7) * 8 + (x & 7))) << kRingSampleBits);
                    const SeedSlot sl = seed_slots<C>(S)[(threadIdx.x & ~63u) + p];
                    st = sl.st;
                    r.dx = sl.u;
                    r.dy = sl.v;
                    Tr = Tg = Tb = (R)1;
                    cr = cg = cb = 0.0;
                    depth = P.max_depth;
                    if (C::COUNT) {
                        cnt.cam_lanes++;
                        t_sample = __builtin_amdgcn_s_memtime();
                    }
                    active = true;
                    new_sample = true;
                }
                blk_next += take;
                need = __ballot(!active);
                continue;
            }
            const unsigned take = min((unsigned)__popcll(need), blk_units - blk_next);
            if (!active && rank < take) {
                const unsigned u = blk_next + rank;
                unsigned si;
                if (nvalid == 64u) {
                    si = u >> 6;
                    x = tx0 + (int)(u & 7u);
                    k = tk0 + (int)((u >> 3) & 7u);
                } else {
                    si = u / nvalid;
                    const unsigned p = u - si * nvalid;
                    x = tx0 + (int)(p % (unsigned)vw);
                    k = tk0 + (int)(p / (unsigned)vw);
                }
                if constexpr (ITEMS) {
                    s = s0 + (int)si * P.spp_chunk;
                    left = min(P.spp, s + P.spp_chunk) - s - 1;
                    cr = cg = cb = 0.0;
                } else {
                    s = s0 + (int)si;
                    if (ring) {
                        if constexpr (!RingSgpr<C>()) cur_slot = (unsigned)__builtin_amdgcn_readlane(ringv, kRingCur);
                        s |= (int)((cur_slot * kRingSlot + si * 64u + (unsigned)((k & 7) * 8 + (x & 7))) << kRingSampleBits);
                    }
                }
                active = true;
                new_sample = true;
            }
            blk_next += take;
            need = __ballot(!active);
        }
        if (!__any(active)) break;
        if (C::COUNT && first_active_lane()) cnt.wave_steps++;
        if (C::COUNT) {
            const uint64_t idle = __ballot(!active);
            if (first_active_lane()) {
                if (exhausted) cnt.idle_tail += (uint32_t)__popcll(idle);
                else cnt.idle_ring += (uint32_t)__popcll(idle);
            }
        }
        if (!active) continue;
        if (C::COUNT) {
            unsigned long long tw = t_prev;
            for (int off = 32; off > 0; off >>= 1) {
                const unsigned long long o = __shfl_xor(tw, off);
                tw = tw > o ? tw : o;
            }
            t_prev = tw;
            RT_STAMP(cnt.t_refill, t_prev);
        }
        bool go = true;
        bool gen_wait = false;
        {
            R u = 0, v = 0;
            bool tries = false;
            if (new_sample) {
                if constexpr (StagedPool<C, ITEMS>()) {
                    u = r.dx;
                    v = r.dy;
                } else if (TryLeft<C>() && cam_wait) {
                    u = r.dx;
                    v = r.dy;
                    cam_wait = false;
                } else {
                    if (C::COUNT) {
                        cnt.cam_lanes++;
                        if (first_active_lane()) cnt.cam_steps++;
                    }
                    int ix, y;
                    image_xy(P, x, k, ix, y);
                    if (C::COUNT) t_sample = __builtin_amdgcn_s_memtime();
                    key.pixel = (uint32_t)y * (uint32_t)P.img_width + (uint32_t)ix;
                    const uint32_t sample = ring ? (uint32_t)s & kRingSampleMask : (uint32_t)s;
                    key.sample = sample;
                    if constexpr (C::F32) ds_start_f32(st, P.seed, key.pixel, sample);
                    else ds_start(st, P.seed, key.pixel, sample);
                    camera_begin(P, ix, y, st, u, v);
                    Tr = Tg = Tb = (R)1;
                    if constexpr (!ITEMS) cr = cg = cb = 0.0;
                    depth = P.max_depth;
                }
                tries = true;
            } else if (pending) {
                tries = shade_draws<C>(S, h.mat);
            }
            RT_STAMP(cnt.t_seed, t_prev);
            R qx = (R)0, qy = (R)0, qz = (R)0, l2 = (R)1;
            const bool three = !new_sample;
            if constexpr (TryLeft<C>()) {
                bool accepted = !tries;
                for (int n = 1;; ++n) {
                    if (!accepted) accepted = unit_try(st, (R)P.scale_m11, three, qx, qy, qz, l2);
                    const uint64_t rejecting = __ballot(!accepted);
                    if (rejecting == 0 || (n >= RT_TRY_MIN && __popcll(rejecting) <= RT_TRY_LEFT)) break;
                }
                gen_wait = !accepted;
            } else {
                while (tries && !unit_try(st, (R)P.scale_m11, three, qx, qy, qz, l2)) {
                }
            }
            RT_STAMP(cnt.t_tries, t_prev);
            if (gen_wait) {
                go = false;
                if (new_sample) {
                    cam_wait = true;
                    r.dx = u;
                    r.dy = v;
                }
            } else if (new_sample) {
                new_sample = false;
                camera_end(P, st, u, v, qx, qy, r);
            } else if (pending) {
                pending = false;
                go = shade_end<C, false>(S, h, r, st, Tr, Tg, Tb, qx, qy, qz, l2);
                if (go) depth -= 1;
            }
        }
        RT_STAMP(t_cam, t_prev);
        if (C::COUNT) {
            cnt.try_wait += gen_wait ? 1u : 0u;
            cnt.no_scatter += (!go && !gen_wait) ? 1u : 0u;
            cnt.depth_cap += (go && depth <= 0) ? 1u : 0u;
        }
        if (go && depth > 0) {
            key.bounce = (uint32_t)(P.max_depth - depth);
            if (C::COUNT) cnt.casts++;
            finish_ray<C>(r, S.has_spheres != 0);
            forget(h);
            RT_STAMP(cnt.t_setup, t_prev);
            const bool hit = trace_world<C>(S, r, h, stack, key, cnt);
            if (C::COUNT) t_prev = __builtin_amdgcn_s_memtime();
            if (!hit) {
                cr = cr + Tr * P.bg[0];
                cg = cg + Tg * P.bg[1];
                cb = cb + Tb * P.bg[2];
            } else {
// ... 91 lines not shown
```

rust-ray-tracing-in-a-weekend_amd/csrc/trace_types.hpp:

```cpp
#pragma once
#include <hip/hip_runtime.h>

#include <algorithm>
#include <type_traits>

#include "rt/rt_numerics.h"
#include "rt/rt_scene.h"
#include "trace_kernel.hpp"

namespace rtk {

typedef float f2v __attribute__((ext_vector_type(2)));
template <class R>
struct RayT {
    R ox, oy, oz;
    R dx, dy, dz;
    R time;
    R a;
    R ya;
    R ix, iy, iz;
    R yx, yy, yz;
    f2v sx, sy, sz;
    uint32_t onx, ony, onz;
};

template <class R>
struct HitT {
    R t, px, py, pz, nx, ny, nz;
    R uv0, uv1, uv2, uv3;
    int front, mat, uvkind;
};
using Hit = HitT<double>;

template <class R>
struct HitRefT {
    R t;
    int prim;
    int sub;
    int side;
};

struct Keyed {
    uint64_t seed;
    uint32_t pixel, sample, bounce;
};

struct Count {
    uint32_t casts, nodes, prims;
    uint32_t wave_steps, wave_nodes;
    uint32_t wave_leaves;
    uint32_t cam_lanes, cam_steps;
    uint32_t shade_lanes, shade_steps;
    uint64_t t_nodes, t_leaves;
    uint64_t t_setup, t_pre, t_rec, t_med, t_inst, t_refill, t_defer;
    uint64_t t_seed, t_tries;
    uint32_t idle_tail, idle_ring, no_scatter, depth_cap, try_wait;
};
#define RT_STAMP(acc, tp)                                                   \
    do {                                                                    \
        if (C::COUNT) {                                                     \
            const uint64_t t_ = __builtin_amdgcn_s_memtime();               \
            if (first_active_lane()) (acc) += t_ - (tp);                    \
            (tp) = t_;                                                      \
        }                                                                   \
    } while (0)
__device__ __forceinline__ bool first_active_lane()
{
    return (int)(threadIdx.x & 63) == __ffsll((long long)__ballot(1)) - 1;
}

#ifndef RT_TRY_LEFT
#define RT_TRY_LEFT 4
#endif
#ifndef RT_TRY_MIN
#define RT_TRY_MIN 2
#endif
template <class C>
constexpr bool TryLeft() { return RT_TRY_LEFT > 0 && (C::F == FEAT_SET_SPHERES || C::F == FEAT_SET_RECTINST); }
template <uint32_t F_, bool S32_, bool LDS_, bool NALL_, bool COUNT_, bool F32_ = false>
struct Cfg {
    static constexpr uint32_t F = F_;
    static constexpr bool S32 = S32_;
    static constexpr bool LDS = LDS_;
    static constexpr bool NALL = NALL_;
    static constexpr bool COUNT = COUNT_;
    static constexpr bool F32 = F32_;
    static constexpr KernelShape SHAPE = kernel_shape(F_, S32_, LDS_, NALL_, F32_);
    static_assert(SHAPE.s32 == S32_ && SHAPE.lds == LDS_ && SHAPE.nall == NALL_ && SHAPE.f32 == F32_, "the shape of this Cfg");
    using Real = typename std::conditional<F32_, float, double>::type;
    static constexpr bool STAGE = false;
};
template <class C>
struct CfgStage : C {
    static constexpr bool STAGE = true;
};

template <class C>
constexpr int BlockThreads() { return C::SHAPE.block_threads; }

template <class C, uint32_t DROP>
struct CfgDrop : C {
    static constexpr uint32_t F = C::F & ~DROP;
};
template <class C, uint32_t DROP>
struct CfgDropStatic : C {
    static constexpr uint32_t F = (C::F & ~DROP) | ((C::F & FEAT_NEST_MOVING) ? 0u : (uint32_t)FEAT_STATIC);
};
template <class C>
using InstC = CfgDropStatic<C, (C::F & FEAT_INST_RECT) ? 0u : (uint32_t)FEAT_RECT>;
template <class C>
using BoundC = CfgDropStatic<C, FEAT_INST_MEDIUM | ((C::F & FEAT_MEDIUM_INST) ? 0u : (uint32_t)(FEAT_RECT | FEAT_INST))>;
template <class C>
using InstMedC = CfgDropStatic<C, FEAT_INST_MEDIUM>;

extern __shared__ int rt_lds[];
__device__ __forceinline__ int lane_remat()
{
    int l;
    asm volatile("v_mbcnt_lo_u32_b32 %0, -1, 0\n\tv_mbcnt_hi_u32_b32 %0, -1, %0" : "=v"(l));
    return l;
}
template <bool LDS, bool REMAT = false, int BT = 256>
struct Stack;
template <int BT>
struct Stack<true, true, BT> {
    int wave0;
    __device__ __forceinline__ int& operator[](int i) const { return rt_lds[wave0 + lane_remat() + i * BT]; }
    __device__ __forceinline__ void init(int stack_off)
    {
        wave0 = stack_off + __builtin_amdgcn_readfirstlane((int)threadIdx.x & ~63);
    }
};
template <int BT>
struct Stack<true, false, BT> {
    int* base;
    __device__ __forceinline__ int& operator[](int i) const { return base[i * BT]; }
    __device__ __forceinline__ void init(int stack_off) { base = rt_lds + stack_off + threadIdx.x; }
};
template <int BT>
struct Stack<false, false, BT> {
    int v[66];
    __device__ __forceinline__ int& operator[](int i) { return v[i]; }
};
template <int BT>
struct Stack16 {
    short* base;
    __device__ __forceinline__ short& operator[](int i) const { return base[i * BT]; }
};
template <class C>
constexpr bool Stack16Cfg() { return C::SHAPE.s16; }
template <class C>
using StackT = typename std::conditional<Stack16Cfg<C>(), Stack16<BlockThreads<C>()>,
                                         Stack<C::LDS, C::LDS && (C::F & FEAT_INST_BLAS) != 0, BlockThreads<C>()>>::type;

__device__ __forceinline__ double rcp_for_div(double b)
{
    const double m = __builtin_fabs(b);
    return (m >= 0x1.0p-900 && m <= 0x1.0p+900) ? 1.0 / b : __builtin_nan("");
}
__device__ __forceinline__ double div_rcp(double q, double b, double y)
{
    const double q0 = q * y;
    const double q1 = __builtin_fma(__builtin_fma(-b, q0, q), y, q0);
    if (__builtin_expect(q1 != q1, 0)) return q / b;
    return q1;
}

__device__ __forceinline__ float f32_inv_dir(double d)
{
    float f = (float)d;
    if (__builtin_fabsf(f) < 1e-30f) f = __builtin_copysignf(1e-30f, f);
    return __builtin_amdgcn_rcpf(f);
}

__device__ __forceinline__ double r_sqrt(double x) { return __builtin_sqrt(x); }
__device__ __forceinline__ float r_sqrt(float x) { return __builtin_sqrtf(x); }
__device__ __forceinline__ double r_fabs(double x) { return __builtin_fabs(x); }
// ... 72 lines not shown
```

rust-ray-tracing-in-a-weekend_amd/rtiow_amd.py:

```python
from __future__ import annotations

import ctypes
import os
from typing import Optional, Sequence

import numpy as np

HERE = os.path.dirname(os.path.abspath(__file__))
LIB_PATH = os.environ.get("RT_LIB_PATH", os.path.join(HERE, "lib", "librtiow_amd.so"))
REPO = os.path.dirname(HERE)
EARTH_JPG = os.path.join(REPO, "assets", "earthmap.jpg")

RT_OK = 0
ERRORS = {-1: "RT_ERR_INVALID", -2: "RT_ERR_HIP", -3: "RT_ERR_UNSUPPORTED", -4: "RT_ERR_OOM",
          -5: "RT_ERR_NO_DEVICE", -6: "RT_ERR_NO_SCENE", -7: "RT_ERR_COMM", -8: "RT_ERR_PEER"}
RT_COMM_ID_BYTES = 128

SCENES = {"random": 0, "two_spheres": 1, "two_perlin": 2, "earth": 3, "simple_light": 4,
          "cornell": 5, "cornell_smoke": 6, "final": 7}
SCENES_NEEDING_IMAGE = (3, 7)

RT_OUT_F32, RT_OUT_F64 = 0, 1
RT_SCHED_CHUNKS = 0
RT_SCHED_POOL = 1
RT_SCHED_ITEMS = 2
RT_SCHED_AUTO = 3
RT_PREC_F64 = 0
RT_PREC_F32 = 1
RT_ACCEL_SAH = 0
RT_ACCEL_LINEAR = 1
RT_ACCEL_MEDIAN = 2
RT_OPT_TRACE_BUF_BYTES = 1
RT_OPT_BATCH_OVERLAP = 2
RT_OPT_BLOCK_SAMPLES = 3
RT_OPT_BLOCK_CHUNKS = 4
RT_OPT_EXTRA_FEATURES = 5
RT_OPT_HOIST = 6
RT_OPT_POOL_RING = 9
RT_OPT_COMM_DIRECT = 10
RT_OPT_AUTO_DEAL_ORDER = 11
RT_BUILD_C_ISECT = 1
RT_BUILD_MAX_LEAF = 2
RT_BUILD_FORCE_LEAF = 3
RT_BUILD_ROOT_LEAF = 4
RT_BUILD_SPLIT_BOX_PAIRS = 5
RT_BUILD_SPLIT_BLAS_PAIRS = 6
RT_BUILD_TIME0 = 7
RT_BUILD_TIME1 = 8

EXPORTED = [
    "rt_abi_version", "rt_last_error", "rt_device_count", "rt_ctx_create", "rt_ctx_destroy",
    "rt_world_create", "rt_world_destroy", "rt_world_texture_solid", "rt_world_texture_checker",
    "rt_world_texture_noise", "rt_world_texture_image", "rt_world_material_lambertian",
    "rt_world_material_metal", "rt_world_material_dielectric", "rt_world_material_diffuse_light",
    "rt_world_material_isotropic", "rt_world_sphere", "rt_world_moving_sphere", "rt_world_rect",
    "rt_world_box", "rt_world_translate", "rt_world_rotate_y", "rt_world_constant_medium",
    "rt_world_bvh", "rt_world_push", "rt_world_build_scene", "rt_world_info_get", "rt_camera_new",
    "rt_scene_preset_get", "rt_scene_camera", "rt_world_flatten", "rt_ctx_upload_soa",
    "rt_ctx_upload_world", "rt_render", "rt_rows_in_shard", "rt_rows_in_band_shard", "rt_tiles_in_shard", "rt_last_stats", "rt_last_counters", "rt_write_ppm",
    "rt_write_ppm_f64", "rt_write_color",
    "rt_ctx_set_variant", "rt_device_eval", "rt_accum_create", "rt_accum_destroy", "rt_accum_add",
    "rt_accum_get", "rt_accum_set", "rt_accum_resolve", "rt_render_progressive", "rt_ctx_set_schedule", "rt_ctx_set_precision",
    "rt_scene_validate", "rt_build_info", "rt_ctx_set_option", "rt_ctx_get_option", "rt_world_set_build_option",
    "rt_last_tile_costs", "rt_ctx_set_tile_order", "rt_last_deal_order",
    "rt_comm_unique_id", "rt_comm_init_rank", "rt_comm_init_all", "rt_comm_destroy", "rt_comm_rank",
    "rt_comm_tile_order", "rt_comm_tile_order_all", "rt_render_gather", "rt_render_gather_all",
    "rt_comm_last_stats", "rt_tiles_assemble", "rt_tiles_assemble_host", "rt_cost_tile_order",
    "rt_render_adaptive", "rt_adaptive_last_stats", "rt_adaptive_tile_errors_host",
    "rt_denoise", "rt_denoise_host", "rt_denoise_last_stats",
    "rt_render_features", "rt_features_last_stats", "rt_denoise_guided", "rt_denoise_guided_host",
    "rt_denoise_atrous", "rt_denoise_atrous_host", "rt_atrous_last_stats",
    "rt_denoise_pyramid", "rt_denoise_pyramid_host", "rt_pyramid_last_stats",
    "rt_render_adaptive_halves", "rt_denoise_cross", "rt_denoise_cross_host", "rt_cross_last_stats",
    "rt_adaptive_state_create", "rt_adaptive_state_destroy", "rt_adaptive_state_advance",
    "rt_adaptive_state_resolve", "rt_adaptive_state_get", "rt_adaptive_state_set",
    "rt_adaptive_state_last_stats", "rt_adaptive_next_group_host",
]

PROGRESS_FN = ctypes.CFUNCTYPE(ctypes.c_int, ctypes.c_void_p, ctypes.c_int64, ctypes.c_int64)


class RTError(RuntimeError):
    pass


class Camera(ctypes.Structure):
    _fields_ = [("origin", ctypes.c_double * 3), ("lower_left_corner", ctypes.c_double * 3),
                ("horizontal", ctypes.c_double * 3), ("vertical", ctypes.c_double * 3),
                ("u", ctypes.c_double * 3), ("v", ctypes.c_double * 3), ("w", ctypes.c_double * 3),
                ("lens_radius", ctypes.c_double), ("time0", ctypes.c_double), ("time1", ctypes.c_double)]


class ScenePreset(ctypes.Structure):
    _fields_ = [("look_from", ctypes.c_double * 3), ("look_at", ctypes.c_double * 3),
                ("background", ctypes.c_double * 3), ("vfov", ctypes.c_double),
                ("aperture", ctypes.c_double), ("focus_dist", ctypes.c_double),
                ("time0", ctypes.c_double), ("time1", ctypes.c_double),
                ("default_width", ctypes.c_int32), ("default_spp", ctypes.c_int32),
                ("default_aspect", ctypes.c_double)]


class WorldInfo(ctypes.Structure):
    _fields_ = [("n_hittables", ctypes.c_int32), ("n_materials", ctypes.c_int32),
                ("n_leaf_prims", ctypes.c_int32), ("n_media", ctypes.c_int32), ("checksum", ctypes.c_double)]


class SceneSoA(ctypes.Structure):
    _fields_ = [("n_prims", ctypes.c_int32), ("n_prim_refs", ctypes.c_int32), ("n_nodes", ctypes.c_int32),
                ("n_instances", ctypes.c_int32), ("n_materials", ctypes.c_int32), ("n_textures", ctypes.c_int32),
                ("n_perlin", ctypes.c_int32), ("n_media", ctypes.c_int32), ("tlas_root", ctypes.c_int32),
                ("accel", ctypes.c_int32), ("image_bytes", ctypes.c_int64), ("pad_extent", ctypes.c_double),
                ("tlas_depth", ctypes.c_int32), ("blas_depth", ctypes.c_int32),
                ("n_tlas_nodes", ctypes.c_int32), ("pad0", ctypes.c_int32),
                ("prims", ctypes.c_void_p), ("prim_refs", ctypes.c_void_p), ("nodes", ctypes.c_void_p),
                ("instances", ctypes.c_void_p), ("materials", ctypes.c_void_p), ("textures", ctypes.c_void_p),
                ("perlin_ranvec", ctypes.c_void_p), ("perlin_perm", ctypes.c_void_p),
                ("image_data", ctypes.c_void_p), ("time_lo", ctypes.c_double), ("time_hi", ctypes.c_double)]


class RenderParams(ctypes.Structure):
    _fields_ = [("width", ctypes.c_int32), ("height", ctypes.c_int32), ("spp", ctypes.c_int32),
                ("max_depth", ctypes.c_int32), ("spp_chunk", ctypes.c_int32), ("row_begin", ctypes.c_int32),
                ("row_stride", ctypes.c_int32), ("out_format", ctypes.c_int32),
                ("out_on_device", ctypes.c_int32), ("count_work", ctypes.c_int32),
                ("background", ctypes.c_double * 3), ("render_seed", ctypes.c_uint64),
                ("stream", ctypes.c_void_p), ("row_block", ctypes.c_int32), ("tile_shard", ctypes.c_int32)]


class Stats(ctypes.Structure):
    _fields_ = [("kernel_ms", ctypes.c_double), ("reduce_ms", ctypes.c_double), ("samples", ctypes.c_uint64),
                ("casts", ctypes.c_uint64), ("node_visits", ctypes.c_uint64), ("prim_tests", ctypes.c_uint64),
                ("n_items", ctypes.c_uint64), ("n_chunks", ctypes.c_int32), ("spp_chunk", ctypes.c_int32),
                ("scene_bytes", ctypes.c_int64), ("node_bytes", ctypes.c_int32), ("prim_bytes", ctypes.c_int32),
                ("material_bytes", ctypes.c_int32), ("variant_features", ctypes.c_int32),
                ("slab32", ctypes.c_int32), ("lds_stack", ctypes.c_int32), ("lds_nodes", ctypes.c_int32),
                ("cycles_camera", ctypes.c_uint64),
                ("cycles_trace", ctypes.c_uint64), ("cycles_shade", ctypes.c_uint64),
                ("wave_steps", ctypes.c_uint64), ("wave_node_steps", ctypes.c_uint64),
                ("cycles_nodes", ctypes.c_uint64), ("cycles_leaves", ctypes.c_uint64),
                ("schedule", ctypes.c_int32), ("n_batches", ctypes.c_int32),
                ("wave_leaf_steps", ctypes.c_uint64), ("camera_lanes", ctypes.c_uint64),
                ("camera_steps", ctypes.c_uint64), ("shade_lanes", ctypes.c_uint64),
                ("shade_steps", ctypes.c_uint64), ("precision", ctypes.c_int32), ("waves_per_simd", ctypes.c_int32),
                ("trace_buf_bytes", ctypes.c_int64), ("overlapped", ctypes.c_int32), ("reserved0", ctypes.c_int32),
                ("ring_bytes", ctypes.c_int64)]

    def as_dict(self):
        return {k: getattr(self, k) for k, _ in self._fields_}


class CommStats(ctypes.Structure):
    _fields_ = [("render_ms", ctypes.c_double), ("gather_ms", ctypes.c_double), ("assemble_ms", ctypes.c_double),
                ("kernel_ms", ctypes.c_double), ("slab_bytes", ctypes.c_int64), ("tiles", ctypes.c_int32),
                ("tile_order", ctypes.c_int32), ("cost_pass_ms", ctypes.c_double), ("peer_failed", ctypes.c_int32)]

    def as_dict(self):
        return {k: getattr(self, k) for k, _ in self._fields_}


class AdaptiveParams(ctypes.Structure):
    _fields_ = [("min_spp", ctypes.c_int32), ("step_spp", ctypes.c_int32), ("threshold", ctypes.c_double)]


class AdaptiveOut(ctypes.Structure):
    _fields_ = [("mean", ctypes.c_void_p), ("tile_spp", ctypes.c_void_p), ("tile_error", ctypes.c_void_p),
                ("stderr_map", ctypes.c_void_p)]


class AdaptiveHalves(ctypes.Structure):
    _fields_ = [("mean_a", ctypes.c_void_p), ("mean_b", ctypes.c_void_p)]


class AdaptiveStats(ctypes.Structure):
    _fields_ = [("passes", ctypes.c_int32), ("min_spp", ctypes.c_int32), ("step_spp", ctypes.c_int32),
                ("spp_chunk", ctypes.c_int32), ("tiles", ctypes.c_int32), ("max_pass_batches", ctypes.c_int32),
                ("samples_traced", ctypes.c_uint64), ("samples_uniform", ctypes.c_uint64),
                ("trace_ms", ctypes.c_double), ("moments_ms", ctypes.c_double), ("classify_ms", ctypes.c_double)]

    def as_dict(self):
        return {k: getattr(self, k) for k, _ in self._fields_}


class AdaptiveAdvanceParams(ctypes.Structure):
    _fields_ = [("threshold", ctypes.c_double), ("spp_cap", ctypes.c_int32), ("max_launches", ctypes.c_int32),
                ("error_on_device", ctypes.c_int32), ("reserved0", ctypes.c_int32),
                ("tile_error_in", ctypes.c_void_p), ("stream", ctypes.c_void_p)]


class AdaptiveStateHeader(ctypes.Structure):
    _fields_ = [("width", ctypes.c_int32), ("height", ctypes.c_int32), ("spp_chunk", ctypes.c_int32),
                ("min_spp", ctypes.c_int32), ("step_spp", ctypes.c_int32), ("with_halves", ctypes.c_int32),
                ("ragged_cap", ctypes.c_int32), ("reserved0", ctypes.c_int32),
                ("groups_total", ctypes.c_uint64), ("samples_total", ctypes.c_uint64)]

    def as_dict(self):
        return {k: getattr(self, k) for k, _ in self._fields_}


class AdaptiveStateData(ctypes.Structure):
    _fields_ = [("sums", ctypes.c_void_p), ("q", ctypes.c_void_p), ("tile_spp", ctypes.c_void_p),
                ("tile_error", ctypes.c_void_p), ("sum_a", ctypes.c_void_p), ("sum_b", ctypes.c_void_p)]


class AdaptiveStateStats(ctypes.Structure):
    _fields_ = [("groups", ctypes.c_int32), ("active_left", ctypes.c_int32), ("min_count", ctypes.c_int32),
                ("max_count", ctypes.c_int32), ("spp_chunk", ctypes.c_int32), ("min_spp", ctypes.c_int32),
                ("step_spp", ctypes.c_int32), ("tiles", ctypes.c_int32), ("samples_traced", ctypes.c_uint64),
                ("groups_total", ctypes.c_uint64), ("samples_total", ctypes.c_uint64),
                ("trace_ms", ctypes.c_double), ("moments_ms", ctypes.c_double), ("classify_ms", ctypes.c_double)]

    def as_dict(self):
        return {k: getattr(self, k) for k, _ in self._fields_}


class AdaptiveGroup(ctypes.Structure):
    _fields_ = [("n_group", ctypes.c_int64), ("n_active", ctypes.c_int64), ("n_star", ctypes.c_int32),
                ("n_next", ctypes.c_int32)]


class DenoiseParams(ctypes.Structure):
    _fields_ = [("width", ctypes.c_int32), ("height", ctypes.c_int32), ("format", ctypes.c_int32),
                ("on_device", ctypes.c_int32), ("radius", ctypes.c_int32), ("patch", ctypes.c_int32),
                ("k", ctypes.c_double), ("stream", ctypes.c_void_p)]


class DenoiseStats(ctypes.Structure):
    _fields_ = [("kernel_ms", ctypes.c_double), ("radius", ctypes.c_int32), ("patch", ctypes.c_int32),
                ("lds_bytes", ctypes.c_int32), ("reserved0", ctypes.c_int32)]

    def as_dict(self):
        return {k: getattr(self, k) for k, _ in self._fields_}
# ... 60 lines not shown
class PyramidStats(ctypes.Structure):
    _fields_ = [("kernel_ms", ctypes.c_double), ("levels", ctypes.c_int32), ("radius", ctypes.c_int32),
                ("patch", ctypes.c_int32), ("reserved0", ctypes.c_int32), ("scratch_bytes", ctypes.c_int64)]

    def as_dict(self):
        return {k: getattr(self, k) for k, _ in self._fields_}


PYRAMID_LEVELS = 3
PYRAMID_WINDOW = (5, 2, 1.0)


CROSS_VARIANCE_SCALE = 2.0

_lib = None


def load_library(path: str = LIB_PATH) -> ctypes.CDLL:
    global _lib
    if _lib is not None:
        return _lib
    if not os.path.exists(path):
        raise RTError(f"HIP library not built: {path} (run __graft_entry__.build())")
    lib = ctypes.CDLL(path)
    P, I, D, U64 = ctypes.c_void_p, ctypes.c_int, ctypes.c_double, ctypes.c_uint64
    PI = ctypes.POINTER(ctypes.c_int)
    PD = ctypes.POINTER(ctypes.c_double)
    sigs = {
        "rt_abi_version": ([], I), "rt_last_error": ([], ctypes.c_char_p), "rt_build_info": ([], ctypes.c_char_p),
        "rt_ctx_set_option": ([P, I, ctypes.c_int64], I),
        "rt_ctx_get_option": ([P, I, ctypes.POINTER(ctypes.c_int64)], I),
        "rt_world_set_build_option": ([P, I, D], I),
        "rt_device_count": ([PI], I), "rt_ctx_create": ([I, ctypes.POINTER(P)], I),
        "rt_ctx_destroy": ([P], None), "rt_world_create": ([U64, ctypes.POINTER(P)], I),
        "rt_world_destroy": ([P], None), "rt_world_texture_solid": ([P, D, D, D, PI], I),
        "rt_world_texture_checker": ([P, PD, PD, PI], I), "rt_world_texture_noise": ([P, D, PI], I),
        "rt_world_texture_image": ([P, P, I, I, PI], I),
        "rt_world_material_lambertian": ([P, I, PI], I), "rt_world_material_metal": ([P, PD, D, PI], I),
        "rt_world_material_dielectric": ([P, D, PI], I), "rt_world_material_diffuse_light": ([P, I, PI], I),
        "rt_world_material_isotropic": ([P, I, PI], I), "rt_world_sphere": ([P, I, PD, D, PI], I),
        "rt_world_moving_sphere": ([P, I, PD, PD, D, D, D, PI], I),
        "rt_world_rect": ([P, I, I, D, D, D, D, D, PI], I), "rt_world_box": ([P, PD, PD, I, PI], I),
        "rt_world_translate": ([P, I, PD, PI], I), "rt_world_rotate_y": ([P, I, D, PI], I),
        "rt_world_constant_medium": ([P, I, D, I, PI], I), "rt_world_bvh": ([P, PI, I, D, D, PI], I),
        "rt_world_push": ([P, I], I), "rt_world_build_scene": ([P, I, P, I, I], I),
        "rt_world_info_get": ([P, ctypes.POINTER(WorldInfo)], I),
        "rt_camera_new": ([PD, PD, PD, D, D, D, D, D, D, ctypes.POINTER(Camera)], I),
        "rt_scene_preset_get": ([I, ctypes.POINTER(ScenePreset)], I),
        "rt_scene_camera": ([I, I, I, ctypes.POINTER(Camera), PD], I),
        "rt_world_flatten": ([P, I, ctypes.POINTER(ctypes.POINTER(SceneSoA))], I),
        "rt_ctx_upload_soa": ([P, ctypes.POINTER(SceneSoA)], I),
        "rt_scene_validate": ([ctypes.POINTER(SceneSoA), ctypes.POINTER(ctypes.c_int32),
                               ctypes.POINTER(ctypes.c_int32)], I), "rt_ctx_upload_world": ([P, P, I], I),
        "rt_render": ([P, ctypes.POINTER(Camera), ctypes.POINTER(RenderParams), P], I),
        "rt_rows_in_shard": ([I, I, I], I), "rt_rows_in_band_shard": ([I, I, I, I], I),
        "rt_tiles_in_shard": ([I, I, I, I], I), "rt_last_stats": ([P, ctypes.POINTER(Stats)], I),
        "rt_last_counters": ([P, P, I], I),
        "rt_last_tile_costs": ([P, P, ctypes.c_int64], I), "rt_ctx_set_tile_order": ([P, P, ctypes.c_int64], I),
        "rt_last_deal_order": ([P, P, ctypes.c_int64], I),
        "rt_write_ppm": ([P, I, I, ctypes.c_char_p], I),
        "rt_write_ppm_f64": ([P, I, I, I, ctypes.c_char_p], I),
        "rt_write_color": ([P, I, ctypes.c_int64, P], I),
        "rt_device_eval": ([P, I, P, P, P, P, I], I), "rt_ctx_set_variant": ([P, I, I, I], I),
        "rt_accum_create": ([P, ctypes.POINTER(RenderParams), ctypes.POINTER(P)], I),
        "rt_ctx_set_schedule": ([P, I], I),
        "rt_ctx_set_precision": ([P, I], I),
        "rt_accum_destroy": ([P], None),
        "rt_accum_add": ([P, P, ctypes.POINTER(Camera), ctypes.POINTER(RenderParams), I], I),
        "rt_accum_get": ([P, P, ctypes.POINTER(ctypes.c_int64)], I),
        "rt_accum_set": ([P, P, ctypes.c_int64], I),
        "rt_accum_resolve": ([P, P, D, I, I, P], I),
        "rt_render_progressive": ([P, ctypes.POINTER(Camera), ctypes.POINTER(RenderParams), I, PROGRESS_FN, P,
                                   P], I),
        "rt_comm_unique_id": ([P], I), "rt_comm_init_rank": ([P, I, I, P, ctypes.POINTER(P)], I),
        "rt_comm_init_all": ([P, I, P], I), "rt_comm_destroy": ([P], None), "rt_comm_rank": ([P, PI, PI], I),
        "rt_comm_tile_order": ([P, ctypes.POINTER(Camera), ctypes.POINTER(RenderParams), I], I),
        "rt_comm_tile_order_all": ([P, I, ctypes.POINTER(Camera), ctypes.POINTER(RenderParams), I], I),
        "rt_render_gather": ([P, ctypes.POINTER(Camera), ctypes.POINTER(RenderParams), P], I),
        "rt_render_gather_all": ([P, I, ctypes.POINTER(Camera), ctypes.POINTER(RenderParams), P], I),
        "rt_comm_last_stats": ([P, ctypes.POINTER(CommStats)], I),
        "rt_tiles_assemble": ([P, P, ctypes.c_int64, I, ctypes.POINTER(RenderParams), P], I),
        "rt_tiles_assemble_host": ([P, ctypes.c_int64, I, I, I, I, P, P], I),
        "rt_cost_tile_order": ([P, ctypes.c_int64, P], I),
        "rt_render_adaptive": ([P, ctypes.POINTER(Camera), ctypes.POINTER(RenderParams),
                                ctypes.POINTER(AdaptiveParams), ctypes.POINTER(AdaptiveOut)], I),
        "rt_render_adaptive_halves": ([P, ctypes.POINTER(Camera), ctypes.POINTER(RenderParams),
                                       ctypes.POINTER(AdaptiveParams), ctypes.POINTER(AdaptiveOut),
                                       ctypes.POINTER(AdaptiveHalves)], I),
        "rt_adaptive_last_stats": ([P, ctypes.POINTER(AdaptiveStats)], I),
        "rt_adaptive_tile_errors_host": ([P, P, P, I, I, P, P], I),
        "rt_denoise": ([P, ctypes.POINTER(DenoiseParams), P, P, P], I),
        "rt_denoise_host": ([ctypes.POINTER(DenoiseParams), P, P, P], I),
        "rt_denoise_last_stats": ([P, ctypes.POINTER(DenoiseStats)], I),
        "rt_render_features": ([P, ctypes.POINTER(Camera), ctypes.POINTER(RenderParams),
                                ctypes.POINTER(FeaturesOut)], I),
        "rt_features_last_stats": ([P, ctypes.POINTER(FeaturesStats)], I),
        "rt_denoise_guided": ([P, ctypes.POINTER(DenoiseParams), P, P, ctypes.POINTER(DenoiseGuides), P], I),
        "rt_denoise_guided_host": ([ctypes.POINTER(DenoiseParams), P, P, ctypes.POINTER(DenoiseGuides), P], I),
        "rt_denoise_atrous": ([P, ctypes.POINTER(AtrousParams), P, P, ctypes.POINTER(DenoiseGuides), P, P], I),
        "rt_denoise_atrous_host": ([ctypes.POINTER(AtrousParams), P, P, ctypes.POINTER(DenoiseGuides), P, P], I),
        "rt_atrous_last_stats": ([P, ctypes.POINTER(AtrousStats)], I),
        "rt_denoise_pyramid": ([P, ctypes.POINTER(PyramidParams), P, P, ctypes.POINTER(DenoiseGuides), P], I),
        "rt_denoise_pyramid_host": ([ctypes.POINTER(PyramidParams), P, P, ctypes.POINTER(DenoiseGuides), P], I),
        "rt_pyramid_last_stats": ([P, ctypes.POINTER(PyramidStats)], I),
        "rt_denoise_cross": ([P, ctypes.POINTER(CrossParams), P, P, P, ctypes.POINTER(DenoiseGuides), P, P], I),
        "rt_denoise_cross_host": ([ctypes.POINTER(CrossParams), P, P, P, ctypes.POINTER(DenoiseGuides), P, P], I),
        "rt_cross_last_stats": ([P, ctypes.POINTER(CrossStats)], I),
        "rt_adaptive_state_create": ([P, ctypes.POINTER(Camera), ctypes.POINTER(RenderParams),
                                      ctypes.POINTER(AdaptiveParams), I, ctypes.POINTER(P)], I),
        "rt_adaptive_state_destroy": ([P], None),
        "rt_adaptive_state_advance": ([P, ctypes.POINTER(AdaptiveAdvanceParams), ctypes.POINTER(ctypes.c_int32)], I),
        "rt_adaptive_state_resolve": ([P, I, I, ctypes.POINTER(AdaptiveOut), ctypes.POINTER(AdaptiveHalves)], I),
        "rt_adaptive_state_get": ([P, ctypes.POINTER(AdaptiveStateHeader), ctypes.POINTER(AdaptiveStateData)], I),
        "rt_adaptive_state_set": ([P, ctypes.POINTER(AdaptiveStateHeader), ctypes.POINTER(AdaptiveStateData)], I),
        "rt_adaptive_state_last_stats": ([P, ctypes.POINTER(AdaptiveStateStats)], I),
        "rt_adaptive_next_group_host": ([P, P, P, ctypes.c_int64, D, ctypes.c_int32, ctypes.c_int32, ctypes.c_int32, P,
                                         ctypes.POINTER(AdaptiveGroup)], I),
    }
    for name, (args, res) in sigs.items():
        fn = getattr(lib, name, None)
        if fn is None:
            continue
        fn.argtypes = args
        fn.restype = res
    _lib = lib
    return lib


def build_info() -> str:
    return load_library().rt_build_info().decode()


def _check(rc: int, what: str) -> None:
    if rc != RT_OK:
        msg = _lib.rt_last_error().decode() if _lib is not None else ""
        raise RTError(f"{what} failed: {ERRORS.get(rc, rc)} {msg}")


def _stats(owner, fn_name: str, Struct):
    s = Struct()
    _check(getattr(owner.lib, fn_name)(owner.h, ctypes.byref(s)), fn_name)
    return s


def _d3(v: Sequence[float]):
    return (ctypes.c_double * 3)(*[float(x) for x in v])


def load_earth_texture(path: str = EARTH_JPG) -> np.ndarray:
    from PIL import Image
    return np.ascontiguousarray(np.asarray(Image.open(path).convert("RGB"), dtype=np.uint8))


class World:

    def __init__(self, scene_seed: int = 1):
        self.lib = load_library()
        h = ctypes.c_void_p()
        _check(self.lib.rt_world_create(ctypes.c_uint64(scene_seed), ctypes.byref(h)), "rt_world_create")
        self.h = h
        self._keep = []

    def close(self):
        if self.h:
            self.lib.rt_world_destroy(self.h)
            self.h = None

    def __del__(self):
        try:
            self.close()
        except Exception:
            pass

    def _id(self, fn, *args) -> int:
        out = ctypes.c_int()
        _check(fn(self.h, *args, ctypes.byref(out)), fn.__name__)
        return out.value

    def solid(self, r, g, b): return self._id(self.lib.rt_world_texture_solid, r, g, b)
    def checker(self, even, odd): return self._id(self.lib.rt_world_texture_checker, _d3(even), _d3(odd))
    def noise(self, scale): return self._id(self.lib.rt_world_texture_noise, scale)

    def image(self, rgb: np.ndarray):
        rgb = np.ascontiguousarray(rgb, dtype=np.uint8)
        return self._id(self.lib.rt_world_texture_image, rgb.ctypes.data, rgb.shape[1], rgb.shape[0])

    def lambertian(self, tex): return self._id(self.lib.rt_world_material_lambertian, tex)
    def metal(self, albedo, fuzz): return self._id(self.lib.rt_world_material_metal, _d3(albedo), fuzz)
    def dielectric(self, ir): return self._id(self.lib.rt_world_material_dielectric, ir)
    def diffuse_light(self, tex): return self._id(self.lib.rt_world_material_diffuse_light, tex)
    def isotropic(self, tex): return self._id(self.lib.rt_world_material_isotropic, tex)

    def sphere(self, mat, center, radius): return self._id(self.lib.rt_world_sphere, mat, _d3(center), radius)

    def moving_sphere(self, mat, c0, c1, t0, t1, radius):
        return self._id(self.lib.rt_world_moving_sphere, mat, _d3(c0), _d3(c1), t0, t1, radius)

    def xy_rect(self, mat, x0, x1, y0, y1, k): return self._id(self.lib.rt_world_rect, 0, mat, x0, x1, y0, y1, k)
    def xz_rect(self, mat, x0, x1, z0, z1, k): return self._id(self.lib.rt_world_rect, 1, mat, x0, x1, z0, z1, k)
    def yz_rect(self, mat, y0, y1, z0, z1, k): return self._id(self.lib.rt_world_rect, 2, mat, y0, y1, z0, z1, k)
    def box(self, mn, mx, mat): return self._id(self.lib.rt_world_box, _d3(mn), _d3(mx), mat)
    def translate(self, child, offset): return self._id(self.lib.rt_world_translate, child, _d3(offset))
    def rotate_y(self, child, angle): return self._id(self.lib.rt_world_rotate_y, child, angle)

    def constant_medium(self, boundary, density, phase):
        return self._id(self.lib.rt_world_constant_medium, boundary, density, phase)

    def bvh(self, ids, t0=0.0, t1=1.0):
        arr = (ctypes.c_int * len(ids))(*ids)
        return self._id(self.lib.rt_world_bvh, arr, len(ids), t0, t1)

    def push(self, hid):
        _check(self.lib.rt_world_push(self.h, hid), "rt_world_push")

    def set_build_option(self, key: int, value: float):
        _check(self.lib.rt_world_set_build_option(self.h, key, float(value)), "rt_world_set_build_option")
        return self

    def build_scene(self, scene_id: int, image: Optional[np.ndarray] = None):
        if scene_id in SCENES_NEEDING_IMAGE and image is None:
            image = load_earth_texture()
        if image is not None:
            image = np.ascontiguousarray(image, dtype=np.uint8)
            self._keep.append(image)
            ptr, w, h = image.ctypes.data, image.shape[1], image.shape[0]
        else:
            ptr, w, h = None, 0, 0
        _check(self.lib.rt_world_build_scene(self.h, scene_id, ptr, w, h), "rt_world_build_scene")
        return self

    def info(self) -> WorldInfo:
        out = WorldInfo()
        _check(self.lib.rt_world_info_get(self.h, ctypes.byref(out)), "rt_world_info_get")
        return out

    def flatten(self, accel: int = RT_ACCEL_SAH) -> SceneSoA:
        p = ctypes.POINTER(SceneSoA)()
        _check(self.lib.rt_world_flatten(self.h, accel, ctypes.byref(p)), "rt_world_flatten")
        return p.contents


def validate_soa(soa: SceneSoA):
    lib = load_library()
    t, b = ctypes.c_int32(), ctypes.c_int32()
    _check(lib.rt_scene_validate(ctypes.byref(soa), ctypes.byref(t), ctypes.byref(b)), "rt_scene_validate")
    return t.value, b.value


def camera_new(look_from, look_at, vup, vfov, aspect_ratio, aperture, focus_dist, time0, time1) -> Camera:
    lib = load_library()
    cam = Camera()
    _check(lib.rt_camera_new(_d3(look_from), _d3(look_at), _d3(vup), vfov, aspect_ratio, aperture, focus_dist,
                             time0, time1, ctypes.byref(cam)), "rt_camera_new")
    return cam


def scene_preset(scene_id: int) -> ScenePreset:
    lib = load_library()
    out = ScenePreset()
    _check(lib.rt_scene_preset_get(scene_id, ctypes.byref(out)), "rt_scene_preset_get")
    return out


def scene_camera(scene_id: int, width: int, height: int):
    lib = load_library()
    cam = Camera()
    bg = (ctypes.c_double * 3)()
    _check(lib.rt_scene_camera(scene_id, width, height, ctypes.byref(cam), bg), "rt_scene_camera")
    return cam, tuple(bg)


def rows_in_shard(height: int, row_begin: int, row_stride: int, row_block: int = 1) -> int:
    if row_block > 1:
        return load_library().rt_rows_in_band_shard(height, row_begin, row_stride, row_block)
    return load_library().rt_rows_in_shard(height, row_begin, row_stride)


def shard_shape(params) -> tuple:
    if params.tile_shard:
        n = tiles_in_shard(params.width, params.height, params.row_begin, params.row_stride)
        return (8 if n else 0), 8 * n
    return rows_in_shard(params.height, params.row_begin, params.row_stride, params.row_block), params.width


def shard_rows(height: int, rank: int, world: int, row_block: int = 1):
    if row_block <= 1:
        return list(range(rank, height, world))
    return [y for band in range(rank, (height + row_block - 1) // row_block, world)
            for y in range(band * row_block, min(height, (band + 1) * row_block))]


def tiles_in_shard(width: int, height: int, tile_begin: int, tile_stride: int) -> int:
    return load_library().rt_tiles_in_shard(width, height, tile_begin, tile_stride)


def _perm(a, axes):
    return a.permute(*axes) if hasattr(a, "permute") else a.transpose(axes)


def cost_tile_order(costs) -> np.ndarray:
    c = np.asarray(costs)
    if c.dtype.kind in "ui" and (c.size == 0 or c.min() >= 0):
        c = np.ascontiguousarray(c, dtype=np.uint64)
        out = np.empty(c.size, dtype=np.uint32)
        _check(load_library().rt_cost_tile_order(c.ctypes.data, c.size, out.ctypes.data), "rt_cost_tile_order")
        return out
    return np.argsort(-np.asarray(c, dtype=np.float64), kind="stable").astype(np.uint32)


def assemble_tiles_host(slabs: np.ndarray, width: int, height: int, world: int, order=None) -> np.ndarray:
    a = np.ascontiguousarray(slabs)
    if a.dtype not in (np.float32, np.float64) or a.ndim < 2 or a.shape[0] != world:
        raise RTError("slabs: world x slab_elems of f32 / f64")
    a = a.reshape(world, -1)
    o = None if order is None else np.ascontiguousarray(order, dtype=np.uint32)
    out = np.zeros((height, width, 3), dtype=a.dtype)
    _check(load_library().rt_tiles_assemble_host(a.ctypes.data, a.shape[1], world, width, height, a.dtype.itemsize,
                                                 None if o is None else o.ctypes.data, out.ctypes.data),
           "rt_tiles_assemble_host")
    return out


def scattered_tile_order(n_tiles: int, stride: int) -> np.ndarray:
    return np.concatenate([np.arange(k, n_tiles, stride) for k in range(stride)]).astype(np.uint32)


def grouped_tile_order(n_tiles: int, world: int, group: int) -> np.ndarray:
    cap = [len(range(r, n_tiles, world)) for r in range(world)]
    lists = [[] for _ in range(world)]
    for j, t0 in enumerate(range(0, n_tiles, group)):
        k = j % world
# ... 834 lines not shown
```

Baseline: 7059.

## Precompute per-pixel primary-ray candidate sphere lists to skip BVH walks

Adds a kernel that bounds each pixel's primary rays, including lens and pixel footprint, with a cone and records up to seven spheres the cone may hit, or a walk flag. The pool trace kernel for the f64 spheres variant reads this 16-byte record per new sample and tests only those candidates instead of traversing the BVH for the first hit. The table is cached per scene upload, camera and params, so later frames skip the build. It costs a 16-byte load per new sample, a larger kernel with more register pressure, and a one-off build with a host sync.

```diff
diff --git a/__graft_entry__.py b/__graft_entry__.py
--- a/__graft_entry__.py
+++ b/__graft_entry__.py
@@ -38,8 +38,8 @@
 SOURCES = ([f"trace_v_{v}.hip" for v in VARIANTS] + [f"trace_v_{v}_count.hip" for v in VARIANTS] +
            [f"trace_f32_{v}.hip" for v in VARIANTS] + ["trace_f32_final_count.hip", "trace_f32_spheres_count.hip"] +
            [f"features_v_{v}.hip" for v in VARIANTS] +
-           ["trace_kernel.hip", "features_kernel.hip", "adaptive_kernel.hip", "adaptive_state_kernel.hip", "denoise_kernel.hip", "atrous_kernel.hip", "cross_kernel.hip", "pyramid_kernel.hip", "scene_model.cpp", "flatten.cpp", "bvh_build.cpp", "scene_lower.cpp",
-            "launch_plan.cpp", "deal_cache.cpp", "denoise_host.cpp", "atrous_host.cpp", "cross_host.cpp", "pyramid_host.cpp", "abi.cpp", "abi_scene.cpp",
+           ["trace_kernel.hip", "features_kernel.hip", "adaptive_kernel.hip", "adaptive_state_kernel.hip", "denoise_kernel.hip", "atrous_kernel.hip", "cross_kernel.hip", "pyramid_kernel.hip", "primary_candidates.hip", "scene_model.cpp", "flatten.cpp", "bvh_build.cpp", "scene_lower.cpp",
+            "launch_plan.cpp", "deal_cache.cpp", "primary_candidates_host.cpp", "denoise_host.cpp", "atrous_host.cpp", "cross_host.cpp", "pyramid_host.cpp", "abi.cpp", "abi_scene.cpp",
             "abi_passes.cpp", "abi_adaptive_state.cpp", "adaptive_frame.cpp", "adaptive_schedule.cpp", "abi_filters.cpp", "comm.cpp"])
 
 
@@ -104,6 +104,7 @@
 SAN_FLAGS = ["-Xarch_host", "-fsanitize=address", "-Xarch_host", "-fsanitize=undefined",
              "-Xarch_host", "-fno-sanitize-recover=undefined", "-Xarch_host", "-fno-omit-frame-pointer"]
 HOST_SOURCES = ["scene_model.cpp", "flatten.cpp", "bvh_build.cpp", "scene_lower.cpp", "launch_plan.cpp", "deal_cache.cpp",
+                "primary_candidates_host.cpp",
                 "denoise_host.cpp", "atrous_host.cpp", "cross_host.cpp", "pyramid_host.cpp", "abi.cpp", "abi_scene.cpp", "abi_passes.cpp",
                 "abi_adaptive_state.cpp", "adaptive_frame.cpp", "adaptive_schedule.cpp", "abi_filters.cpp",
                 "comm.cpp"]
diff --git a/include/rt/rt_abi.h b/include/rt/rt_abi.h
--- a/include/rt/rt_abi.h
+++ b/include/rt/rt_abi.h
@@ -159,8 +159,20 @@
     int32_t overlapped;
     int32_t reserved0;
     int64_t ring_bytes;
+    int64_t primary_table_bytes;
+    double primary_build_ms;
+    double primary_walk_share;
 } rt_stats;
 int rt_last_stats(rt_ctx* ctx, rt_stats* out);
+
+typedef struct rt_primary_candidates_info {
+    int64_t pixels, flagged;
+    int64_t candidates;
+    int32_t max_candidates;
+    int32_t slots;
+} rt_primary_candidates_info;
+int rt_primary_candidates_host(const rt_scene_soa* scene, const rt_camera* cam, int width, int height, int k_max,
+                               uint16_t* records, rt_primary_candidates_info* info);
 int rt_last_counters(rt_ctx* ctx, uint64_t* out, int n);
 
 int rt_last_tile_costs(rt_ctx* ctx, uint64_t* out, int64_t n);
@@ -438,7 +450,9 @@
     RT_OPT_HOIST = 6,
     RT_OPT_POOL_RING = 9,
     RT_OPT_COMM_DIRECT = 10,
-    RT_OPT_AUTO_DEAL_ORDER = 11
+    RT_OPT_AUTO_DEAL_ORDER = 11,
+    RT_OPT_PRIMARY_CANDIDATES = 12,
+    RT_OPT_PRIMARY_CANDIDATES_K = 13
 };
 int rt_ctx_set_option(rt_ctx* ctx, int key, int64_t value);
 int rt_ctx_get_option(rt_ctx* ctx, int key, int64_t* value);
diff --git a/rust-ray-tracing-in-a-weekend_amd/csrc/abi.cpp b/rust-ray-tracing-in-a-weekend_amd/csrc/abi.cpp
--- a/rust-ray-tracing-in-a-weekend_amd/csrc/abi.cpp
+++ b/rust-ray-tracing-in-a-weekend_amd/csrc/abi.cpp
@@ -12,6 +12,7 @@
 #include "ctx_internal.hpp"
 #include "deal_cache.hpp"
 #include "launch_plan.hpp"
+#include "primary_candidates.hpp"
 #include "render_internal.hpp"
 #include "scene_lower.hpp"
 #include "trace_kernel.hpp"
@@ -99,6 +100,7 @@
     if (e == hipSuccess) e = c->ev_in.create(hipEventDisableTiming);
     if (e == hipSuccess) e = c->ev_tr.create(hipEventDisableTiming);
     if (e == hipSuccess) e = c->ev_rd.create(hipEventDisableTiming);
+    if (e == hipSuccess) e = c->ev_pc.create();
     if (e == hipSuccess) e = c->counters.alloc(kCounters * sizeof(unsigned long long));
     if (e == hipSuccess) e = c->params.alloc(kParamSlots * sizeof(rtk::KParams));
     if (e == hipSuccess) e = c->work.alloc(2 * rtk::kDealTable * sizeof(unsigned));
@@ -133,6 +135,7 @@
     if (rc) return fail(rc, err);
     c->upload_gen++;
     c->deal.drop();
+    c->primary_valid = false;
     c->last_deal_n = 0;
 
     struct Table {
@@ -316,6 +319,46 @@
         K.tile_major = rtk::kDealOrdered;
         c->last_deal_n = img_tiles;
     }
+    return RT_OK;
+}
+
+static int primary_setup(rt_ctx* c, const rt_camera* cam, const rt_render_params* p, const rtp::Plan& pl, bool count_work,
+                         hipStream_t stream, rtk::KParams& K, rtk::LaunchOpts& o)
+{
+    rt_stats& st = c->stats;
+    st.primary_table_bytes = 0;
+    st.primary_build_ms = 0.0;
+    st.primary_walk_share = 0.0;
+    const size_t bytes = rtpc::table_bytes(p->width, p->height);
+    if (!c->opt_primary || pl.variant != rtk::FEAT_SET_SPHERES || pl.f32 || pl.schedule != RT_SCHED_POOL || !pl.shape.s16 ||
+        pl.seed_stage_bytes == 0 || count_work || bytes > rtpc::kMaxTableBytes || p->width < 2 || p->height < 2)
+        return RT_OK;
+    rtd::Key key = rtd::key_of(c->upload_gen, *cam, *p);
+    key.row_begin = 0;
+    key.row_stride = key.row_block = 1;
+    if (!(c->primary_valid && rtd::same_key(key, c->primary_key) && c->primary_k == c->opt_primary_k)) {
+        c->primary_valid = false;
+        int rc = c->primary_tab.reserve(stream, bytes + 16);
+        if (rc) return rc;
+        unsigned* const flagged = reinterpret_cast<unsigned*>(c->primary_tab.as<char>() + bytes);
+        HIP_TRY(c->ev_pc.record(0, stream));
+        HIP_TRY(rtk::launch_primary_candidates(c->S, *cam, p->width, p->height, c->opt_primary_k, c->primary_tab.p, flagged, stream));
+        HIP_TRY(c->ev_pc.record(1, stream));
+        unsigned n_flagged = 0;
+        HIP_TRY(hipMemcpyAsync(&n_flagged, flagged, sizeof n_flagged, hipMemcpyDeviceToHost, stream));
+        HIP_TRY(hipStreamSynchronize(stream));
+        float ms = 0.0f;
+        HIP_TRY(c->ev_pc.elapsed(0, &ms));
+        c->primary_key = key;
+        c->primary_k = c->opt_primary_k;
+        c->primary_flagged = (int64_t)n_flagged;
+        c->primary_valid = true;
+        st.primary_build_ms = ms;
+    }
+    K.primary = c->primary_tab.as<uint4>();
+    o.primary = 1;
+    st.primary_table_bytes = (int64_t)bytes;
+    st.primary_walk_share = (double)c->primary_flagged / ((double)p->width * (double)p->height);
     return RT_OK;
 }
 
@@ -407,6 +450,8 @@
     o.waves_per_simd = &waves_per_simd;
     const rtk::SampleTiles tiles{lay.w, lay.rows, (lay.w + 7) / 8, pl.f32};
     rc = deal_setup(c, cam, p, pl, sink.moments != nullptr, img_tiles, stream, K);
+    if (rc) return rc;
+    rc = primary_setup(c, cam, p, pl, rq.count_work, stream, K, o);
     if (rc) return rc;
 
     if (pl.own_total) HIP_TRY(hipMemsetAsync(acc, 0, pl.px_bytes, stream));
@@ -803,6 +848,14 @@
         if (v < 0 || v > 2) return fail(RT_ERR_INVALID, "deal order mode out of range (0 off, 1 auto, 2 measure only)");
         c->opt_deal = (int)v;
         return RT_OK;
+    case RT_OPT_PRIMARY_CANDIDATES:
+        if (v < 0 || v > 1) return fail(RT_ERR_INVALID, "primary candidates out of range (0 off, 1 on)");
+        c->opt_primary = (int)v;
+        return RT_OK;
+    case RT_OPT_PRIMARY_CANDIDATES_K:
+        if (v < 1 || v > rtpc::kSlots) return fail(RT_ERR_INVALID, "primary candidates per pixel out of range (1..7)");
+        c->opt_primary_k = (int)v;
+        return RT_OK;
     default: return fail(RT_ERR_INVALID, "unknown option");
     }
 }
@@ -820,6 +873,8 @@
     case RT_OPT_POOL_RING: *v = c->opt.ring; return RT_OK;
     case RT_OPT_COMM_DIRECT: *v = c->opt_comm_direct; return RT_OK;
     case RT_OPT_AUTO_DEAL_ORDER: *v = c->opt_deal; return RT_OK;
+    case RT_OPT_PRIMARY_CANDIDATES: *v = c->opt_primary; return RT_OK;
+    case RT_OPT_PRIMARY_CANDIDATES_K: *v = c->opt_primary_k; return RT_OK;
     default: return fail(RT_ERR_INVALID, "unknown option");
     }
 }
diff --git a/rust-ray-tracing-in-a-weekend_amd/csrc/abi_scene.cpp b/rust-ray-tracing-in-a-weekend_amd/csrc/abi_scene.cpp
--- a/rust-ray-tracing-in-a-weekend_amd/csrc/abi_scene.cpp
+++ b/rust-ray-tracing-in-a-weekend_amd/csrc/abi_scene.cpp
@@ -8,6 +8,7 @@
 #include "rt/rt_abi.h"
 #include "rt/rt_numerics.h"
 #include "ctx_internal.hpp"
+#include "primary_candidates.hpp"
 #include "scene_lower.hpp"
 #include "scene_model.hpp"
 
@@ -302,6 +303,27 @@
     return RT_OK;
 }
 
+int rt_primary_candidates_host(const rt_scene_soa* s, const rt_camera* cam, int width, int height, int k_max,
+                               uint16_t* records, rt_primary_candidates_info* info)
+{
+    if (!s || !cam || !records || width < 1 || height < 1 || k_max < 1) return fail(RT_ERR_INVALID, "bad argument");
+    rtl::Lowered L;
+    std::string err;
+    const int rc = rtl::lower(*s, true, L, err);
+    if (rc) return fail(rc, err);
+    static_assert(sizeof(rtpc::Record) == 8 * sizeof(uint16_t), "a record is 8 uint16");
+    const rtpc::TableStats st = rtpc::build_host(L.nodes.data(), L.leaf_prims.data(), s->tlas_root, *cam, width, height, k_max,
+                                                 reinterpret_cast<rtpc::Record*>(records));
+    if (info) {
+        info->pixels = st.pixels;
+        info->flagged = st.flagged;
+        info->candidates = st.candidates;
+        info->max_candidates = st.max_candidates;
+        info->slots = rtpc::kSlots;
+    }
+    return RT_OK;
+}
+
 static inline int write_color_f64(double x, double scale)
 {
     const double r = std::sqrt(x * scale);
diff --git a/rust-ray-tracing-in-a-weekend_amd/csrc/ctx_internal.hpp b/rust-ray-tracing-in-a-weekend_amd/csrc/ctx_internal.hpp
--- a/rust-ray-tracing-in-a-weekend_amd/csrc/ctx_internal.hpp
+++ b/rust-ray-tracing-in-a-weekend_amd/csrc/ctx_internal.hpp
@@ -172,6 +172,14 @@
     rtd::DealCache deal;
     int64_t deal_cap = 0;
     int64_t last_deal_n = 0;
+    int opt_primary = 1;
+    int opt_primary_k = 7;
+    DevBuf primary_tab;
+    bool primary_valid = false;
+    rtd::Key primary_key;
+    int primary_k = 0;
+    int64_t primary_flagged = 0;
+    EventSpan<2> ev_pc;
 };
 
 struct StreamScope {
diff --git a/rust-ray-tracing-in-a-weekend_amd/csrc/primary_candidates.hip b/rust-ray-tracing-in-a-weekend_amd/csrc/primary_candidates.hip
--- /dev/null
+++ b/rust-ray-tracing-in-a-weekend_amd/csrc/primary_candidates.hip
@@ -0,0 +1,42 @@
+#include "primary_candidates.hpp"
+#include "trace_kernel.hpp"
+
+namespace rtk {
+
+__global__ void __launch_bounds__(256) primary_candidates(const rt_bvh_node* __restrict__ nodes,
+                                                          const rt_prim* __restrict__ leaf_prims, int32_t root, rt_camera cam,
+                                                          int width, int height, int k_max, uint4* __restrict__ table,
+                                                          unsigned* __restrict__ flagged)
+{
+    const long long i = (long long)blockIdx.x * blockDim.x + threadIdx.x;
+    const long long n = (long long)width * height;
+    bool walk = false;
+    if (i < n) {
+        const int y = (int)(i / width), ix = (int)(i - (long long)y * width);
+        const rtpc::Record r = rtpc::build_pixel(nodes, leaf_prims, root, rtpc::cone_of(cam, width, height, ix, y), k_max);
+        uint4 q;
+        q.x = (unsigned)r.n | (unsigned)r.slot[0] << 16;
+        q.y = (unsigned)r.slot[1] | (unsigned)r.slot[2] << 16;
+        q.z = (unsigned)r.slot[3] | (unsigned)r.slot[4] << 16;
+        q.w = (unsigned)r.slot[5] | (unsigned)r.slot[6] << 16;
+        table[i] = q;
+        walk = r.n == rtpc::kWalk;
+    }
+    const unsigned long long m = __ballot(walk);
+    if (m != 0 && (threadIdx.x & 63u) == (unsigned)(__ffsll((long long)m) - 1)) atomicAdd(flagged, (unsigned)__popcll(m));
+}
+
+hipError_t launch_primary_candidates(const SceneDev& S, const rt_camera& cam, int width, int height, int k_max, void* table,
+                                     unsigned* flagged, hipStream_t stream)
+{
+    const long long n = (long long)width * height;
+    if (n <= 0) return hipSuccess;
+    const hipError_t e = hipMemsetAsync(flagged, 0, sizeof(unsigned), stream);
+    if (e != hipSuccess) return e;
+    if (k_max > rtpc::kSlots) k_max = rtpc::kSlots;
+    hipLaunchKernelGGL(primary_candidates, dim3((unsigned)((n + 255) / 256)), dim3(256), 0, stream, S.nodes, S.leaf_prims,
+                       S.tlas_root, cam, width, height, k_max, (uint4*)table, flagged);
+    return hipGetLastError();
+}
+
+}
diff --git a/rust-ray-tracing-in-a-weekend_amd/csrc/primary_candidates.hpp b/rust-ray-tracing-in-a-weekend_amd/csrc/primary_candidates.hpp
--- /dev/null
+++ b/rust-ray-tracing-in-a-weekend_amd/csrc/primary_candidates.hpp
@@ -0,0 +1,171 @@
+#pragma once
+
+#include <cstddef>
+#include <cstdint>
+
+#include "rt/rt_scene.h"
+
+#ifdef __HIPCC__
+#include <hip/hip_runtime.h>
+#define RT_PC_HD __host__ __device__ inline
+#else
+#define RT_PC_HD inline
+#endif
+
+namespace rtpc {
+
+constexpr int kSlots = 7;
+constexpr uint16_t kWalk = 0xffff;
+struct Record {
+    uint16_t n;
+    uint16_t slot[kSlots];
+};
+static_assert(sizeof(Record) == 16, "one 16-byte load per new sample");
+
+constexpr size_t kMaxTableBytes = (size_t)256 << 20;
+constexpr double kMaxSlope = 0.5;
+constexpr int kSweepPieces = 32;
+constexpr int kStack = 64;
+
+struct Cone {
+    double o[3], d[3];
+    double dd;
+    double lr, hd;
+    double shrink;
+    double time_lo, time_hi;
+    bool covered;
+};
+
+RT_PC_HD double dot3(const double* a, const double* b) { return a[0] * b[0] + a[1] * b[1] + a[2] * b[2]; }
+RT_PC_HD bool is_fin(double x) { return x - x == 0.0; }
+
+RT_PC_HD Cone cone_of(const rt_camera& cam, int width, int height, int ix, int y)
+{
+    Cone c;
+    const double su = ((double)ix + 0.5) / ((double)width - 1.0), sv = ((double)y + 0.5) / ((double)height - 1.0);
+    double hh = 0.0, vv = 0.0;
+    for (int a = 0; a < 3; ++a) {
+        c.o[a] = cam.origin[a];
+        c.d[a] = cam.lower_left_corner[a] + cam.horizontal[a] * su + cam.vertical[a] * sv - cam.origin[a];
+        hh += cam.horizontal[a] * cam.horizontal[a];
+        vv += cam.vertical[a] * cam.vertical[a];
+    }
+    c.dd = dot3(c.d, c.d);
+    c.hd = 0.5 * (__builtin_sqrt(hh) / ((double)width - 1.0) + __builtin_sqrt(vv) / ((double)height - 1.0));
+    const double uu = dot3(cam.u, cam.u), vv2 = dot3(cam.v, cam.v), uv = __builtin_fabs(dot3(cam.u, cam.v));
+    c.lr = __builtin_fabs(cam.lens_radius) * __builtin_sqrt((uu > vv2 ? uu : vv2) + uv);
+    c.time_lo = cam.time0 < cam.time1 ? cam.time0 : cam.time1;
+    c.time_hi = cam.time0 < cam.time1 ? cam.time1 : cam.time0;
+    const double k = (c.lr + c.hd) / __builtin_sqrt(c.dd);
+    c.covered = width > 1 && height > 1 && c.dd > 0.0 && is_fin(c.dd) && is_fin(c.lr) && is_fin(c.hd) && k <= kMaxSlope &&
+                is_fin(c.time_lo) && is_fin(c.time_hi);
+    c.shrink = c.covered ? __builtin_sqrt(1.0 - k * k) : 0.0;
+    return c;
+}
+
+RT_PC_HD bool may_hit_ball(const Cone& c, const double* centre, double radius)
+{
+    const double w[3] = {centre[0] - c.o[0], centre[1] - c.o[1], centre[2] - c.o[2]};
+    double t = dot3(w, c.d) / c.dd;
+    if (!(t > 0.0)) t = 0.0;
+    const double q[3] = {w[0] - t * c.d[0], w[1] - t * c.d[1], w[2] - t * c.d[2]};
+    const double dist = __builtin_sqrt(dot3(q, q));
+    const double cone_r = __builtin_fabs(1.0 - t) * c.lr + t * c.hd;
+    const double reach = radius + cone_r;
+    const double margin = 1e-7 * (1.0 + reach + dist);
+    return !(dist * c.shrink > reach + margin);
+}
+
+enum Verdict { kMiss = 0, kMay = 1, kUnknown = 2 };
+
+RT_PC_HD Verdict may_hit_prim(const Cone& c, const rt_prim& p)
+{
+    const double rho = __builtin_fabs(p.p[3]);
+    if (p.kind == RT_PRIM_SPHERE) return may_hit_ball(c, p.p, rho) ? kMay : kMiss;
+    if (p.kind != RT_PRIM_MOVING_SPHERE) return kUnknown;
+    double s0 = c.time_lo, s1 = c.time_hi;
+    if (!(p.p[8] == 0.0 && p.p[9] == 1.0)) {
+        s0 = (c.time_lo - p.p[8]) / (p.p[9] - p.p[8]);
+        s1 = (c.time_hi - p.p[8]) / (p.p[9] - p.p[8]);
+    }
+    const double speed = __builtin_sqrt(p.p[5] * p.p[5] + p.p[6] * p.p[6] + p.p[7] * p.p[7]);
+    const double half = 0.5 * __builtin_fabs(s1 - s0) * speed;
+    if (!is_fin(half) || !is_fin(s0) || !is_fin(s1)) return kMay;
+    int pieces = 1;
+    while (pieces < kSweepPieces && half > 0.25 * rho * (double)pieces) pieces *= 2;
+    const double ds = (s1 - s0) / (double)pieces, piece = half / (double)pieces;
+    for (int i = 0; i < pieces; ++i) {
+        const double sm = s0 + ((double)i + 0.5) * ds;
+        const double mid[3] = {p.p[0] + p.p[5] * sm, p.p[1] + p.p[6] * sm, p.p[2] + p.p[7] * sm};
+        if (may_hit_ball(c, mid, rho + piece + 1e-9 * (1.0 + piece + half))) return kMay;
+    }
+    return kMiss;
+}
+
+RT_PC_HD bool may_hit_box(const Cone& c, const float* lo, const float* hi)
+{
+    double mid[3], h2 = 0.0;
+    for (int a = 0; a < 3; ++a) {
+        mid[a] = 0.5 * ((double)lo[a] + (double)hi[a]);
+        const double h = 0.5 * ((double)hi[a] - (double)lo[a]);
+        h2 += h * h;
+    }
+    if (!is_fin(h2) || !is_fin(mid[0]) || !is_fin(mid[1]) || !is_fin(mid[2])) return true;
+    return may_hit_ball(c, mid, __builtin_sqrt(h2));
+}
+
+RT_PC_HD Record build_pixel(const rt_bvh_node* nodes, const rt_prim* leaf_prims, int32_t root, const Cone& c, int k_max)
+{
+    Record r;
+    r.n = 0;
+    for (int i = 0; i < kSlots; ++i) r.slot[i] = 0;
+    if (!c.covered) {
+        r.n = kWalk;
+        return r;
+    }
+    int32_t stack[kStack];
+    int sp = 0;
+    int32_t cur = root;
+    for (;;) {
+        if (cur >= 0) {
+            const rt_bvh_node& nd = nodes[cur];
+            const bool h0 = may_hit_box(c, nd.lo0, nd.hi0), h1 = may_hit_box(c, nd.lo1, nd.hi1);
+            if (h0 && h1) {
+                if (sp == kStack) {
+                    r.n = kWalk;
+                    return r;
+                }
+                stack[sp++] = nd.child[1];
+                cur = nd.child[0];
+                continue;
+            }
+            if (h0 || h1) {
+                cur = h0 ? nd.child[0] : nd.child[1];
+                continue;
+            }
+        } else {
+            const int32_t code = ~cur, first = code >> 5, count = cur == INT32_MIN ? 0 : code & 31;
+            for (int32_t j = first; j < first + count; ++j) {
+                const Verdict v = may_hit_prim(c, leaf_prims[j]);
+                if (v == kMiss) continue;
+                if (v == kUnknown || (int)r.n >= k_max || j >= (int32_t)kWalk) {
+                    r.n = kWalk;
+                    return r;
+                }
+                r.slot[r.n++] = (uint16_t)j;
+            }
+        }
+        if (sp == 0) return r;
+        cur = stack[--sp];
+    }
+}
+
+struct TableStats {
+    int64_t pixels = 0, flagged = 0, candidates = 0;
+    int max_candidates = 0;
+};
+TableStats build_host(const rt_bvh_node* nodes, const rt_prim* leaf_prims, int32_t root, const rt_camera& cam, int width,
+                      int height, int k_max, Record* out);
+inline size_t table_bytes(int width, int height) { return (size_t)width * (size_t)height * sizeof(Record); }
+
+}
diff --git a/rust-ray-tracing-in-a-weekend_amd/csrc/primary_candidates_host.cpp b/rust-ray-tracing-in-a-weekend_amd/csrc/primary_candidates_host.cpp
--- /dev/null
+++ b/rust-ray-tracing-in-a-weekend_amd/csrc/primary_candidates_host.cpp
@@ -0,0 +1,26 @@
+#include "primary_candidates.hpp"
+
+namespace rtpc {
+
+TableStats build_host(const rt_bvh_node* nodes, const rt_prim* leaf_prims, int32_t root, const rt_camera& cam, int width,
+                      int height, int k_max, Record* out)
+{
+    TableStats st;
+    if (k_max > kSlots) k_max = kSlots;
+    for (int y = 0; y < height; ++y) {
+        for (int ix = 0; ix < width; ++ix) {
+            const Record r = build_pixel(nodes, leaf_prims, root, cone_of(cam, width, height, ix, y), k_max);
+            out[(size_t)y * (size_t)width + (size_t)ix] = r;
+            st.pixels++;
+            if (r.n == kWalk) {
+                st.flagged++;
+            } else {
+                st.candidates += r.n;
+                if ((int)r.n > st.max_candidates) st.max_candidates = (int)r.n;
+            }
+        }
+    }
+    return st;
+}
+
+}
diff --git a/rust-ray-tracing-in-a-weekend_amd/csrc/trace_kernel.hip b/rust-ray-tracing-in-a-weekend_amd/csrc/trace_kernel.hip
--- a/rust-ray-tracing-in-a-weekend_amd/csrc/trace_kernel.hip
+++ b/rust-ray-tracing-in-a-weekend_amd/csrc/trace_kernel.hip
@@ -253,6 +253,7 @@
     L.pool = o.pool;
     L.waves_per_simd = o.waves_per_simd;
     L.max_waves = o.pool == 1 && Ph.ring ? (unsigned)Ph.ring_waves : 0u;
+    L.primary = o.primary != 0 && Ph.primary != nullptr;
     const long long groups = o.pool == 2   ? (Ph.n_chunks + std::max(1, Ph.block_chunks) - 1) / std::max(1, Ph.block_chunks)
                              : o.pool == 1 ? ((long long)Ph.spp - Ph.sample_begin + std::max(1, Ph.block_samples) - 1) /
                                                  std::max(1, Ph.block_samples)
diff --git a/rust-ray-tracing-in-a-weekend_amd/csrc/trace_kernel.hpp b/rust-ray-tracing-in-a-weekend_amd/csrc/trace_kernel.hpp
--- a/rust-ray-tracing-in-a-weekend_amd/csrc/trace_kernel.hpp
+++ b/rust-ray-tracing-in-a-weekend_amd/csrc/trace_kernel.hpp
@@ -62,6 +62,7 @@
     int32_t tile_major;
     uint32_t deal_div;
     unsigned long long* tile_cost;
+    const uint4* primary;
 };
 
 constexpr int32_t kDealOrdered = 2, kDealMeasure = 3;
@@ -75,6 +76,7 @@
     int count;
     int pool;
     int f32;
+    int primary = 0;
     int* waves_per_simd = nullptr;
 };
 
@@ -127,6 +129,8 @@
 
 hipError_t launch_trace(const SceneDev& S, const KParams& Ph, const KParams* P, double* out,
                         unsigned long long* counters, unsigned* work, const LaunchOpts& o, hipStream_t stream);
+hipError_t launch_primary_candidates(const SceneDev& S, const rt_camera& cam, int width, int height, int k_max, void* table,
+                                     unsigned* flagged, hipStream_t stream);
 hipError_t launch_reduce_samples(const double* samples, void* out, bool f64, SampleTiles g, int n_samples,
                                  int chunk, double scale, hipStream_t stream);
 hipError_t launch_reduce_samples_carry(const double* samples, double* acc, double* open, SampleTiles g,
diff --git a/rust-ray-tracing-in-a-weekend_amd/csrc/trace_launch.hpp b/rust-ray-tracing-in-a-weekend_amd/csrc/trace_launch.hpp
--- a/rust-ray-tracing-in-a-weekend_amd/csrc/trace_launch.hpp
+++ b/rust-ray-tracing-in-a-weekend_amd/csrc/trace_launch.hpp
@@ -19,6 +19,11 @@
                     if constexpr (RT_STAGE_SEEDS != 0 && C::SHAPE.s16)
                         return any_static_lds({(const void*)trace_pool<CfgStage<C>, false>, (const void*)trace_pool<CfgStage<C>, false, true>});
                     else return false;
+                }() ||
+                [] {
+                    if constexpr (RT_STAGE_SEEDS != 0 && C::SHAPE.s16 && F == FEAT_SET_SPHERES && !COUNT)
+                        return any_static_lds({(const void*)trace_pool<CfgPrimary<C>, false>, (const void*)trace_pool<CfgPrimary<C>, false, true>});
+                    else return false;
                 }();
             if (static_lds) k = without_stack16(k);
         }
@@ -36,6 +41,10 @@
                 if (L.max_waves) nb = std::max(1u, std::min(nb, L.max_waves / (unsigned)wpb));
                 hipLaunchKernelGGL(kernel, dim3(nb), dim3(bt), lds, stream, S, L.P, L.out, L.counters, L.work);
             };
+            if constexpr (RT_STAGE_SEEDS != 0 && C1::SHAPE.s16 && !F32 && F == FEAT_SET_SPHERES && !COUNT) {
+                if (seed_bytes && L.primary)
+                    return go(L.max_waves ? trace_pool<CfgPrimary<C1>, false, true> : trace_pool<CfgPrimary<C1>, false>);
+            }
             if constexpr (RT_STAGE_SEEDS != 0 && C1::SHAPE.s16 && !F32) {
                 if (seed_bytes) return go(L.max_waves ? trace_pool<CfgStage<C1>, false, true> : trace_pool<CfgStage<C1>, false>);
             }
diff --git a/rust-ray-tracing-in-a-weekend_amd/csrc/trace_launch_common.hpp b/rust-ray-tracing-in-a-weekend_amd/csrc/trace_launch_common.hpp
--- a/rust-ray-tracing-in-a-weekend_amd/csrc/trace_launch_common.hpp
+++ b/rust-ray-tracing-in-a-weekend_amd/csrc/trace_launch_common.hpp
@@ -13,6 +13,7 @@
     unsigned long long n_blocks;
     int* waves_per_simd;
     unsigned max_waves = 0;
+    bool primary = false;
 };
 
 template <class K>
diff --git a/rust-ray-tracing-in-a-weekend_amd/csrc/trace_pool.hpp b/rust-ray-tracing-in-a-weekend_amd/csrc/trace_pool.hpp
--- a/rust-ray-tracing-in-a-weekend_amd/csrc/trace_pool.hpp
+++ b/rust-ray-tracing-in-a-weekend_amd/csrc/trace_pool.hpp
@@ -95,6 +95,101 @@
             p += (size_t)NB * 64 * 3;
         }
         if (own) o[c] = a;
+    }
+}
+
+template <class C, bool ITEMS>
+constexpr bool PrimaryPool()
+{
+    static_assert(!C::PRIMARY || (C::STAGE && !C::COUNT && C::F == FEAT_SET_SPHERES && TryLeft<C>()),
+                  "primary candidates: the f64 spheres variant's timed staged kernels");
+    return C::PRIMARY && StagedPool<C, ITEMS>();
+}
+template <class C, class R = typename C::Real>
+__device__ __forceinline__ void generate_primary(const SceneDev& S, const KParams& P, int x, int k, int& depth, bool& new_sample,
+                                                 bool& pending, rt_pstream& st, RayT<R>& r, HitT<R>& h, R& Tr, R& Tg, R& Tb,
+                                                 double& cr, double& cg, double& cb, bool& go, bool& gen_wait, Count& cnt)
+{
+    go = false;
+    if (__any(new_sample)) {
+        uint4 rec = make_uint4(0xffffu, 0u, 0u, 0u);
+        if (new_sample) {
+            int ix, y;
+            image_xy(P, x, k, ix, y);
+            if ((unsigned)ix < (unsigned)P.img_width && (unsigned)y < (unsigned)P.height)
+                rec = P.primary[(size_t)y * (size_t)P.img_width + (size_t)ix];
+        }
+        R qx = (R)0, qy = (R)0, qz = (R)0, l2 = (R)1;
+        bool accepted = !new_sample;
+        for (int n = 1;; ++n) {
+            if (!accepted) accepted = unit_try(st, (R)P.scale_m11, false, qx, qy, qz, l2);
+            const uint64_t rejecting = __ballot(!accepted);
+            if (rejecting == 0 || (n >= RT_TRY_MIN && __popcll(rejecting) <= RT_TRY_LEFT)) break;
+        }
+        unsigned n_cand = 0;
+        if (new_sample && !accepted) {
+            gen_wait = true;
+        } else if (new_sample) {
+            new_sample = false;
+            const R u = r.dx, v = r.dy;
+            camera_end(P, st, u, v, qx, qy, r);
+            const unsigned n = rec.x & 0xffffu;
+            if (n > 7u || depth <= 0) go = true;
+            else {
+                finish_ray<C, false>(r, true);
+                n_cand = n + 1;
+            }
+        }
+        if (__any(n_cand != 0)) {
+            const R t_min = (R)0.001;
+            R t_max = (R)RT_INF;
+            HitRefT<R> best;
+            best.sub = 0;
+            best.side = 0;
+            best.prim = -1;
+            uint64_t a = ((uint64_t)rec.y << 32 | (uint64_t)rec.x) >> 16;
+            const uint64_t b = (uint64_t)rec.w << 32 | (uint64_t)rec.z;
+#pragma unroll 1
+            for (unsigned i = 0; __ballot(i + 1 < n_cand) != 0; ++i) {
+                if (i + 1 < n_cand) {
+                    const int slot = (int)((unsigned)a & 0xffffu);
+                    if (simple_t<C>(S.leaf_prims[slot], r, t_min, t_max, best.t, best.side, cnt, false)) {
+                        best.prim = slot;
+                        t_max = best.t;
+                    }
+                }
+                a >>= 16;
+                if (i == 2) a = b;
+            }
+            if (n_cand != 0) {
+                if (best.prim < 0) {
+                    cr = cr + Tr * P.bg[0];
+                    cg = cg + Tg * P.bg[1];
+                    cb = cb + Tb * P.bg[2];
+                } else {
+                    finish_hit<C>(S, r, best, h);
+                    pending = shade_begin<C>(S, h, Tr, Tg, Tb, cr, cg, cb);
+                }
+            }
+        }
+    }
+    if (__any(pending)) {
+        R qx = (R)0, qy = (R)0, qz = (R)0, l2 = (R)1;
+        bool accepted = !(pending && shade_draws<C>(S, h.mat));
+        for (int n = 1;; ++n) {
+            if (!accepted) accepted = unit_try(st, (R)P.scale_m11, true, qx, qy, qz, l2);
+            const uint64_t rejecting = __ballot(!accepted);
+            if (rejecting == 0 || (n >= RT_TRY_MIN && __popcll(rejecting) <= RT_TRY_LEFT)) break;
+        }
+        if (pending) {
+            if (!accepted) {
+                gen_wait = true;
+            } else {
+                pending = false;
+                go = shade_end<C, false>(S, h, r, st, Tr, Tg, Tb, qx, qy, qz, l2);
+                if (go) depth -= 1;
+            }
+        }
     }
 }
 
@@ -370,7 +465,9 @@
         }
         bool go = true;
         bool gen_wait = false;
-        {
+        if constexpr (PrimaryPool<C, ITEMS>())
+            generate_primary<C>(S, P, x, k, depth, new_sample, pending, st, r, h, Tr, Tg, Tb, cr, cg, cb, go, gen_wait, cnt);
+        if constexpr (!PrimaryPool<C, ITEMS>()) {
             R u = 0, v = 0;
             bool tries = false;
             if (new_sample) {
diff --git a/rust-ray-tracing-in-a-weekend_amd/csrc/trace_types.hpp b/rust-ray-tracing-in-a-weekend_amd/csrc/trace_types.hpp
--- a/rust-ray-tracing-in-a-weekend_amd/csrc/trace_types.hpp
+++ b/rust-ray-tracing-in-a-weekend_amd/csrc/trace_types.hpp
@@ -89,10 +89,16 @@
     static_assert(SHAPE.s32 == S32_ && SHAPE.lds == LDS_ && SHAPE.nall == NALL_ && SHAPE.f32 == F32_, "the shape of this Cfg");
     using Real = typename std::conditional<F32_, float, double>::type;
     static constexpr bool STAGE = false;
+    static constexpr bool PRIMARY = false;
 };
 template <class C>
 struct CfgStage : C {
     static constexpr bool STAGE = true;
+};
+
+template <class C>
+struct CfgPrimary : CfgStage<C> {
+    static constexpr bool PRIMARY = true;
 };
 
 template <class C>
diff --git a/rust-ray-tracing-in-a-weekend_amd/rtiow_amd.py b/rust-ray-tracing-in-a-weekend_amd/rtiow_amd.py
--- a/rust-ray-tracing-in-a-weekend_amd/rtiow_amd.py
+++ b/rust-ray-tracing-in-a-weekend_amd/rtiow_amd.py
@@ -39,6 +39,8 @@
 RT_OPT_POOL_RING = 9
 RT_OPT_COMM_DIRECT = 10
 RT_OPT_AUTO_DEAL_ORDER = 11
+RT_OPT_PRIMARY_CANDIDATES = 12
+RT_OPT_PRIMARY_CANDIDATES_K = 13
 RT_BUILD_C_ISECT = 1
 RT_BUILD_MAX_LEAF = 2
 RT_BUILD_FORCE_LEAF = 3
@@ -75,6 +77,7 @@
     "rt_adaptive_state_create", "rt_adaptive_state_destroy", "rt_adaptive_state_advance",
     "rt_adaptive_state_resolve", "rt_adaptive_state_get", "rt_adaptive_state_set",
     "rt_adaptive_state_last_stats", "rt_adaptive_next_group_host",
+    "rt_primary_candidates_host",
 ]
 
 PROGRESS_FN = ctypes.CFUNCTYPE(ctypes.c_int, ctypes.c_void_p, ctypes.c_int64, ctypes.c_int64)
@@ -143,10 +146,17 @@
                 ("camera_steps", ctypes.c_uint64), ("shade_lanes", ctypes.c_uint64),
                 ("shade_steps", ctypes.c_uint64), ("precision", ctypes.c_int32), ("waves_per_simd", ctypes.c_int32),
                 ("trace_buf_bytes", ctypes.c_int64), ("overlapped", ctypes.c_int32), ("reserved0", ctypes.c_int32),
-                ("ring_bytes", ctypes.c_int64)]
+                ("ring_bytes", ctypes.c_int64),
+                ("primary_table_bytes", ctypes.c_int64), ("primary_build_ms", ctypes.c_double),
+                ("primary_walk_share", ctypes.c_double)]
 
     def as_dict(self):
         return {k: getattr(self, k) for k, _ in self._fields_}
+
+
+class PrimaryCandidatesInfo(ctypes.Structure):
+    _fields_ = [("pixels", ctypes.c_int64), ("flagged", ctypes.c_int64), ("candidates", ctypes.c_int64),
+                ("max_candidates", ctypes.c_int32), ("slots", ctypes.c_int32)]
 
 
 class CommStats(ctypes.Structure):
@@ -373,6 +383,8 @@
         "rt_tiles_assemble": ([P, P, ctypes.c_int64, I, ctypes.POINTER(RenderParams), P], I),
         "rt_tiles_assemble_host": ([P, ctypes.c_int64, I, I, I, I, P, P], I),
         "rt_cost_tile_order": ([P, ctypes.c_int64, P], I),
+        "rt_primary_candidates_host": ([ctypes.POINTER(SceneSoA), ctypes.POINTER(Camera), I, I, I, P,
+                                        ctypes.POINTER(PrimaryCandidatesInfo)], I),
         "rt_render_adaptive": ([P, ctypes.POINTER(Camera), ctypes.POINTER(RenderParams),
                                 ctypes.POINTER(AdaptiveParams), ctypes.POINTER(AdaptiveOut)], I),
         "rt_render_adaptive_halves": ([P, ctypes.POINTER(Camera), ctypes.POINTER(RenderParams),
@@ -538,6 +550,14 @@
     return t.value, b.value
 
 
+def primary_candidates_host(soa: SceneSoA, cam: Camera, width: int, height: int, k_max: int = 7):
+    rec = np.zeros((height, width, 8), dtype=np.uint16)
+    info = PrimaryCandidatesInfo()
+    _check(load_library().rt_primary_candidates_host(ctypes.byref(soa), ctypes.byref(cam), width, height, k_max,
+                                                     rec.ctypes.data, ctypes.byref(info)), "rt_primary_candidates_host")
+    return rec, info
+
+
 def camera_new(look_from, look_at, vup, vfov, aspect_ratio, aperture, focus_dist, time0, time1) -> Camera:
     lib = load_library()
     cam = Camera()
```

Result: faster. 7541 (median of 6 runs) (+6.8%).
